# LSaldyt/JAX_llama

Measured on AMD Instinct MI355X. Metric: output_tokens_per_sec, higher is better.
Workload: dtype bf16; 1 GPU; model=llama3-8b, global_batch=2048, seq_len=384, prompt_len=128, gen_len=256, parallelism=dp1, mp=1

## Files before the change

### jax_llama_amd/csrc/bindings.cpp

```cpp
#include <torch/extension.h>
#include <c10/hip/HIPStream.h>

#include "kernels/launchers.h"

namespace {

using torch::Tensor;

hipStream_t stream() { return c10::hip::getCurrentHIPStream().stream(); }

void check(bool cond, const char* msg) { TORCH_CHECK(cond, "jax_llama_amd._C: ", msg); }

void check_gpu(const Tensor& t, const char* name) {
  TORCH_CHECK(t.is_cuda(), "jax_llama_amd._C: ", name, " must be a GPU tensor");
  TORCH_CHECK(t.is_contiguous(), "jax_llama_amd._C: ", name, " must be contiguous");
}

void rc(int r, const char* what) {
  TORCH_CHECK(r == 0, "jax_llama_amd._C: ", what, " failed (code ", r, ")");
}

void gemm_rc(int r, const char* what) {
  const char* why = r == -1   ? "no legal plan for this shape / tile id / epilogue / fused norm / K split"
                    : r == -3 ? "the slab workspace is missing or too small"
// ... 311 lines not shown
                     int64_t splits, c10::optional<Tensor> x_packed, int64_t spl, c10::optional<Tensor> sk_ws,
                     c10::optional<Tensor> sk_tk, c10::optional<Tensor> o_w, int64_t o_n, int64_t o_k,
                     c10::optional<Tensor> o_h, c10::optional<Tensor> o_hb, c10::optional<Tensor> o_hb_pack,
                     int64_t tp_state) {
  check_gpu(x, "x");
  check_packed(w, n, k);
  check(x.dim() == 2 && x.size(1) == k && x.scalar_type() == torch::kBFloat16, "linear_qkv_attn: x bf16 [M, K]");
  const int64_t m = x.size(0);
  check(m <= 32, "linear_qkv_attn: M <= 32");
  jla::QKVArgs qa = qkv_args(m, n, table, positions, kc, vc, slot, 1, h, hkv, dh, q);
  for (auto* t : {&kv_start, &out, &ws, &tickets, &sync}) check_gpu(*t, "linear_qkv_attn arg");
  check(kv_start.scalar_type() == torch::kInt32 && kv_start.numel() == m, "kv_start int32 [B]");
  check(out.scalar_type() == torch::kBFloat16 && out.numel() == m * h * dh, "out bf16 [B, H * Dh]");
  check(ws.scalar_type() == torch::kFloat32 && ws.numel() >= m * hkv * splits * (h / hkv) * (dh + 4), "ws too small");
  check(tickets.scalar_type() == torch::kInt32 && tickets.numel() >= m * hkv, "tickets int32 [pairs]");
  check(sync.scalar_type() == torch::kInt32 && (size_t)sync.numel() >= jla::qkv_attn_sync_ints(),
        "sync int32 [qkv_attn_sync_ints()]");
  check(t_cap <= kc.size(2), "t_cap <= cache length");
  const jla::bf16_t* xp = packed_ptr(x_packed, m, k, "x_packed");
  check(spl == 1 || spl == 2, "linear_qkv_attn: spl 1 or 2");
  if (spl > 1) {
    check(sk_ws.has_value() && sk_tk.has_value(), "linear_qkv_attn spl 2: sk_ws and sk_tk (skinny_workspace)");
    check_gpu(*sk_ws, "sk_ws");
    check_gpu(*sk_tk, "sk_tk");
    check(sk_ws->scalar_type() == torch::kFloat32 && sk_tk->scalar_type() == torch::kInt32 &&
              sk_tk->numel() >= n / 16,
          "linear_qkv_attn: sk_ws fp32, sk_tk int32 [N / 16]");
    qa.sk_ws = ptr<float>(*sk_ws);
    qa.sk_tk = ptr<int32_t>(*sk_tk);
    qa.sk_ws_floats = (int)sk_ws->numel();
  }
  jla::QKVArgs qo{};
  float* oh = nullptr;
  int o_mode = 0;
  if (o_w.has_value()) {
    check_packed(*o_w, o_n, o_k);
    check(o_k == h * dh, "linear_qkv_attn: Wo has H * Dh input columns");
    check(o_h.has_value() && o_hb.has_value(), "linear_qkv_attn: the fused o projection needs h and hb");
    check_gpu(*o_h, "h");
    check_gpu(*o_hb, "hb");
    check(o_h->scalar_type() == torch::kFloat32 && o_h->numel() == m * o_n && o_hb->scalar_type() == torch::kBFloat16 &&
              o_hb->numel() == m * o_n, "linear_qkv_attn: h fp32 / hb bf16 [M, N_o]");
    const int og = jla::qkv_attn_o_groups((int)m, (int)(h / hkv), (int)o_n, (int)o_k);
    check(og > 0, "linear_qkv_attn: the o projection cannot be fused at this shape (qkv_attn_o_groups)");
    oh = ptr<float>(*o_h);
    qo.res_bf16 = bf(*o_hb);
    qo.pack = packed_ptr(o_hb_pack, m, o_n, "o_hb_pack");
    o_mode = MODE_RESIDUAL;
    if (tp_state) {
      void* st = reinterpret_cast<void*>(tp_state);
      check(og <= jla::CAR_WG_COUNTERS && og * jla::TPRES_REGION <= jla::car_max_bytes(st),
            "linear_qkv_attn: too many o workgroups for the TP buffer");
      qo.tp = jla::car_device(st);
      o_mode = MODE_TPRESID;
    }
  }
  rc(jla::linear_qkv_attn(xp ? xp : cbf(x), w.data_ptr(), m, n, k, (float)rms_eps, qa, xp != nullptr, bf(out),
                          packed_ptr(out_pack, m, h * dh, "out_pack"), ptr<int32_t>(kv_start), ptr<float>(ws),
                          ptr<int32_t>(tickets), ptr<int32_t>(sync), (int)t_cap, (int)splits, (int)spl, stream(),
                          o_w.has_value() ? o_w->data_ptr() : nullptr, oh, (int)o_n, (int)o_k, o_mode,
                          o_w.has_value() ? &qo : nullptr),
     "linear_qkv_attn");
}

bool check_gemm_ws(const c10::optional<Tensor>& ws, int64_t k, int64_t ksplit, int64_t m, int64_t n, bool rms,
                   int64_t tile) {
  if (!is_g5(tile) && ksplit <= 1) return false;
  check(ws.has_value(), "gemm: a K split (gemm5: any plan) needs the slab workspace");
  check_gpu(*ws, "gemm ws");
  const int64_t ks = is_g5(tile) ? jla::gemm5_ksplit((int)k, (int)ksplit) : ksplit;
  check(ws->scalar_type() == torch::kFloat32 && ws->numel() >= ks * m * (n + (rms ? 1 : 0)), "gemm ws too small");
  return true;
}

static float* rms_ws_ptr(const c10::optional<Tensor>& rws, int64_t m, size_t* floats) {
  *floats = 0;
  if (!rws.has_value()) return nullptr;
  check_gpu(*rws, "rms_ws");
  check(rws->scalar_type() == torch::kFloat32 && rws->numel() >= m, "rms_ws: fp32, >= M floats");
  *floats = rws->numel();
  return ptr<float>(*rws);
}

void gemm(Tensor x, Tensor w, int64_t n, int64_t k, Tensor out, int64_t mode, bool accumulate,
          c10::optional<Tensor> mirror, int64_t ksplit, c10::optional<Tensor> ws, double rms_eps, int64_t tile,
          c10::optional<Tensor> pack_out, c10::optional<Tensor> rms_ws, int64_t n_body) {
  check_gpu(x, "x");
  check_packed(w, n, k);
  check(n_body >= 0 && (n_body == 0 || jla::gemm_tail_width((int)tile) > 0), "gemm n_body: tail-balanced tiles only");
  check(x.dim() == 2 && x.size(1) == k && x.scalar_type() == torch::kBFloat16, "x must be bf16 [M, K]");
  check(mode >= 0 && mode <= 2, "gemm mode");
  const int64_t m = x.size(0);
  check_linear_out(out, m, n, mode);
  jla::bf16_t* mir = mode == 1 ? mirror_ptr(mirror, out.numel()) : nullptr;
  jla::QKVArgs pqa{};
  if (pack_out.has_value()) {
    check(m <= SKINNY_MAX_M && (mode == 1 || mode == 2) && (mode != 1 || mir), "gemm pack_out: decode M, residual "
          "(with its mirror) or SwiGLU");
    check(ksplit > 1 || is_g5(tile), "gemm pack_out: the split-K reduce-kernel path only");
    pqa.pack = packed_ptr(pack_out, m, mode == 2 ? n / 2 : n, "pack_out");
  }
  const bool slabs = check_gemm_ws(ws, k, ksplit, m, n, rms_eps >= 0, tile);
  size_t rfl = 0;
  float* rws = rms_ws_ptr(rms_ws, m, &rfl);
  gemm_rc(jla::gemm(cbf(x), w.data_ptr(), out.data_ptr(), m, n, k, mode, accumulate,
                    out.scalar_type() == torch::kFloat32, mir, pqa.pack ? &pqa : nullptr,
                    slabs ? ptr<float>(*ws) : nullptr, slabs ? ws->numel() : 0, ksplit, stream(), (float)rms_eps,
                    (int)tile, rws, rfl, (int)n_body),
          "gemm");
}

void gemm_qkv(Tensor x, Tensor w, int64_t n, int64_t k, Tensor table, Tensor positions, Tensor kc, Tensor vc,
              Tensor slot, int64_t seq_len, int64_t h, int64_t hkv, int64_t dh, Tensor q, int64_t ksplit,
              c10::optional<Tensor> ws, double rms_eps, int64_t tile, c10::optional<Tensor> rms_ws) {
  check_gpu(x, "x");
  check_packed(w, n, k);
  check(x.dim() == 2 && x.size(1) == k && x.scalar_type() == torch::kBFloat16, "x must be bf16 [M, K]");
  const int64_t m = x.size(0);
  jla::QKVArgs qa = qkv_args(m, n, table, positions, kc, vc, slot, seq_len, h, hkv, dh, q);
  const bool slabs = check_gemm_ws(ws, k, ksplit, m, n, rms_eps >= 0, tile);
  size_t rfl = 0;
  float* rws = rms_ws_ptr(rms_ws, m, &rfl);
  gemm_rc(jla::gemm(cbf(x), w.data_ptr(), nullptr, m, n, k, MODE_QKV, 0, 0, nullptr, &qa,
                    slabs ? ptr<float>(*ws) : nullptr, slabs ? ws->numel() : 0, ksplit, stream(), (float)rms_eps,
                    (int)tile, rws, rfl),
          "gemm_qkv");
}

void rope_kv_write(Tensor qkv, Tensor table, Tensor positions, Tensor kc, Tensor vc, Tensor slot, int64_t seq_len,
                   int64_t h, int64_t hkv, int64_t dh, Tensor q) {
  for (auto* t : {&qkv, &table, &positions, &kc, &vc, &slot, &q}) check_gpu(*t, "rope_kv_write arg");
  check(qkv.scalar_type() == torch::kBFloat16 && kc.scalar_type() == torch::kBFloat16 &&
            vc.scalar_type() == torch::kBFloat16 && q.scalar_type() == torch::kBFloat16,
        "rope_kv_write bf16 tensors");
  check(table.scalar_type() == torch::kFloat32 && table.dim() == 3 && table.size(1) == dh / 2 && table.size(2) == 2,
        "rope table must be fp32 [L, Dh/2, 2]");
  check(positions.scalar_type() == torch::kInt32 && slot.scalar_type() == torch::kInt32, "int32 positions/slot");
  const int64_t m = qkv.size(0);
  check(qkv.dim() == 2 && qkv.size(1) == (h + 2 * hkv) * dh, "qkv shape");
  check(positions.numel() == m && m % seq_len == 0, "positions shape");
  const int64_t b = m / seq_len;
  check(kc.dim() == 4 && kc.size(0) == b && kc.size(1) == hkv && kc.size(3) == dh && vc.sizes() == kc.sizes(),
        "cache shape [B, Hkv, T, Dh]");
  check(q.numel() == m * h * dh, "q out shape");
  rc(jla::rope_kv_write(cbf(qkv), ptr<float>(table), table.size(0), ptr<int32_t>(positions), bf(kc), bf(vc),
                        ptr<int32_t>(slot), m, seq_len, h, hkv, dh, kc.size(2), bf(q), stream()),
     "rope_kv_write");
}

void check_attn(const Tensor& q, const Tensor& kc, const Tensor& vc, const Tensor& slot, const Tensor& kv_start,
                const c10::optional<Tensor>& key_mask, const Tensor& out) {
  for (auto* t : {&q, &kc, &vc, &slot, &kv_start, &out}) check_gpu(*t, "attention arg");
  check(q.scalar_type() == torch::kBFloat16 && kc.scalar_type() == torch::kBFloat16 &&
            vc.scalar_type() == torch::kBFloat16 && out.scalar_type() == torch::kBFloat16,
        "attention bf16 tensors");
  check(q.dim() == 4 && kc.dim() == 4 && kc.sizes() == vc.sizes(), "attention shapes");
  check(kc.size(0) == q.size(0) && kc.size(3) == q.size(3), "cache/q shape mismatch");
  check(q.size(2) % kc.size(1) == 0, "H must be a multiple of Hkv");
  check(slot.scalar_type() == torch::kInt32 && kv_start.scalar_type() == torch::kInt32 &&
            kv_start.numel() == q.size(0),
        "slot/kv_start");
  check(out.numel() == q.numel(), "attention out shape");
  if (key_mask.has_value()) {
    check_gpu(*key_mask, "key_mask");
    check(key_mask->scalar_type() == torch::kUInt8 && key_mask->dim() == 2 && key_mask->size(0) == q.size(0),
          "key_mask must be uint8 [B, L]");
  }
}

void attn_decode(Tensor q, Tensor kc, Tensor vc, Tensor slot, Tensor kv_start, c10::optional<Tensor> key_mask,
                 Tensor out, Tensor ws, Tensor tickets, int64_t t_cap, int64_t nsplit, c10::optional<Tensor> out_pack) {
  check_attn(q, kc, vc, slot, kv_start, key_mask, out);
  check(q.size(1) == 1, "attn_decode: one query per row");
  const int64_t b = q.size(0), h = q.size(2), dh = q.size(3), hkv = kc.size(1), T = kc.size(2);
  check(t_cap <= T, "t_cap exceeds the cache length");
  check_gpu(ws, "ws");
  check_gpu(tickets, "tickets");
  const jla::AttnPlanResult r = jla::attn_decode_plan(jla::attn_knobs(), b, h, hkv, dh, t_cap, key_mask.has_value());
  TORCH_CHECK(r.rc == 0, "jax_llama_amd._C: attn_decode: no plan (", r.why, "; see attn_plan.h)");
  TORCH_CHECK(nsplit == r.plan.nsplit, "jax_llama_amd._C: attn_decode: nsplit ", nsplit, " is not the plan's ",
              r.plan.nsplit, " (attn_decode_plan_check)");
  check(!out_pack.has_value() || r.plan.packs,
        "attn_decode: this launch does not write the packed copy (attn_decode_plan_check's packs)");
  check(ws.scalar_type() == torch::kFloat32 && (size_t)ws.numel() >= r.plan.ws_floats, "workspace too small");
  check(tickets.scalar_type() == torch::kInt32 && tickets.numel() >= r.plan.tickets, "tickets too small");
  const uint8_t* km = key_mask.has_value() ? ptr<uint8_t>(*key_mask) : nullptr;
  const int ml = key_mask.has_value() ? key_mask->size(1) : 0;
  rc(jla::attn_decode(cbf(q), cbf(kc), cbf(vc), ptr<int32_t>(slot), ptr<int32_t>(kv_start), km, ml, bf(out),
                      ptr<float>(ws), ptr<int32_t>(tickets), b, h, hkv, dh, T, t_cap, nsplit, stream(),
                      packed_ptr(out_pack, b, h * dh, "out_pack")),
     "attn_decode");
}

void attn_prefill(Tensor q, Tensor kc, Tensor vc, Tensor slot, Tensor kv_start, c10::optional<Tensor> key_mask,
                  Tensor out) {
  check_attn(q, kc, vc, slot, kv_start, key_mask, out);
  const uint8_t* km = key_mask.has_value() ? ptr<uint8_t>(*key_mask) : nullptr;
  const int ml = key_mask.has_value() ? key_mask->size(1) : 0;
  rc(jla::attn_prefill(cbf(q), cbf(kc), cbf(vc), ptr<int32_t>(slot), ptr<int32_t>(kv_start), km, ml, bf(out),
                       q.size(0), q.size(1), q.size(2), kc.size(1), q.size(3), kc.size(2), stream()),
     "attn_prefill");
}

void argmax(Tensor logits, Tensor idx, Tensor val) {
  check_gpu(logits, "logits");
  check_gpu(idx, "idx");
  check_gpu(val, "val");
  check(logits.scalar_type() == torch::kFloat32 && logits.dim() == 2, "logits must be fp32 [B, V]");
  check(idx.scalar_type() == torch::kInt32 && val.scalar_type() == torch::kFloat32 &&
            idx.numel() == logits.size(0) && val.numel() == logits.size(0),
        "argmax outputs");
  rc(jla::argmax(ptr<float>(logits), logits.size(0), logits.size(1), ptr<int32_t>(idx), ptr<float>(val), stream()),
     "argmax");
}

void gemm_argmax(Tensor x, Tensor w, int64_t n, int64_t k, Tensor ws, double rms_eps, Tensor idx, Tensor val,
                 c10::optional<Tensor> rms_ws) {
  check_gpu(x, "x");
  check_packed(w, n, k);
  check(x.dim() == 2 && x.size(1) == k && x.scalar_type() == torch::kBFloat16, "x must be bf16 [M, K]");
  const int64_t m = x.size(0);
  check_gpu(ws, "ws");
  check(ws.scalar_type() == torch::kFloat32 && (size_t)ws.numel() >= jla::gemm_argmax_workspace_floats(m, n),
        "gemm_argmax ws too small");
  check_gpu(idx, "idx");
  check_gpu(val, "val");
  check(idx.scalar_type() == torch::kInt32 && val.scalar_type() == torch::kFloat32 && idx.numel() == m &&
            val.numel() == m,
        "gemm_argmax outputs");
  size_t rfl = 0;
  float* rws = rms_ws_ptr(rms_ws, m, &rfl);
  rc(jla::gemm_argmax(cbf(x), w.data_ptr(), ptr<float>(ws), ws.numel(), m, n, k, (float)rms_eps, ptr<int32_t>(idx),
                      ptr<float>(val), stream(), rws, rfl),
     "gemm_argmax");
}

static void check_logprob_io(const Tensor& targets, const Tensor& tgt, const Tensor& mx, const Tensor& se, int64_t m,
                             int64_t col_offset) {
  for (auto* t : {&targets, &tgt, &mx, &se}) check_gpu(*t, "logprob arg");
  check(targets.scalar_type() == torch::kInt32 && targets.numel() == m, "targets must be int32 [M]");
  for (auto* t : {&tgt, &mx, &se})
    check(t->scalar_type() == torch::kFloat32 && t->numel() == m, "logprob outputs must be fp32 [M]");
  check(col_offset >= 0 && col_offset <= INT32_MAX, "col_offset");
}

void gemm_logprob(Tensor x, Tensor w, int64_t n, int64_t k, Tensor ws, double rms_eps, Tensor targets,
                  int64_t col_offset, Tensor tgt, Tensor mx, Tensor se, c10::optional<Tensor> rms_ws) {
  check_gpu(x, "x");
  check_packed(w, n, k);
  check(x.dim() == 2 && x.size(1) == k && x.scalar_type() == torch::kBFloat16, "x must be bf16 [M, K]");
  const int64_t m = x.size(0);
  check_gpu(ws, "ws");
  check(ws.scalar_type() == torch::kFloat32 && (size_t)ws.numel() >= jla::gemm_logprob_workspace_floats(m, n),
        "gemm_logprob ws too small");
  check_logprob_io(targets, tgt, mx, se, m, col_offset);
  size_t rfl = 0;
  float* rws = rms_ws_ptr(rms_ws, m, &rfl);
  gemm_rc(jla::gemm_logprob(cbf(x), w.data_ptr(), ptr<float>(ws), ws.numel(), m, n, k, (float)rms_eps,
                            ptr<int32_t>(targets), (int)col_offset, ptr<float>(tgt), ptr<float>(mx), ptr<float>(se),
                            stream(), rws, rfl),
          "gemm_logprob");
}

void logprob_rows(Tensor logits, Tensor targets, int64_t col_offset, Tensor tgt, Tensor mx, Tensor se) {
  check_gpu(logits, "logits");
  check(logits.scalar_type() == torch::kFloat32 && logits.dim() == 2 && logits.size(1) > 0,
        "logits must be fp32 [B, V]");
  check(logits.size(1) <= INT32_MAX, "logprob_rows: V too large");
  check_logprob_io(targets, tgt, mx, se, logits.size(0), col_offset);
  rc(jla::logprob_rows(ptr<float>(logits), logits.size(0), logits.size(1), ptr<int32_t>(targets), (int)col_offset,
                       ptr<float>(tgt), ptr<float>(mx), ptr<float>(se), stream()),
     "logprob_rows");
}

void topk_chunk(Tensor logits, int64_t k, int64_t idx_offset, Tensor cv, Tensor ci) {
  for (auto* t : {&logits, &cv, &ci}) check_gpu(*t, "topk_chunk arg");
  check(logits.scalar_type() == torch::kFloat32 && logits.dim() == 2, "logits must be fp32 [B, V]");
  const int64_t b = logits.size(0), v = logits.size(1);
  check(k >= 1 && k <= 64 && k <= v, "topk_chunk: 1 <= k <= min(64, V)");
  const int64_t c = (int64_t)jla::topk_chunks(v) * k;
  check(cv.scalar_type() == torch::kFloat32 && ci.scalar_type() == torch::kInt32 && cv.numel() == b * c &&
            ci.numel() == b * c,
        "topk_chunk: candidates must be [B, chunks*k] fp32/int32");
  rc(jla::topk_chunk(ptr<float>(logits), b, v, k, idx_offset, ptr<float>(cv), ptr<int32_t>(ci), stream()),
     "topk_chunk");
}

void topk_merge(Tensor cv, Tensor ci, int64_t k, int64_t mode, c10::optional<Tensor> out_v,
                c10::optional<Tensor> out_i, c10::optional<Tensor> nxt, double temperature, double top_p,
                int64_t seed, c10::optional<Tensor> step) {
  check_gpu(cv, "cv");
  check_gpu(ci, "ci");
  check(cv.dim() == 2 && cv.sizes() == ci.sizes() && cv.scalar_type() == torch::kFloat32 &&
            ci.scalar_type() == torch::kInt32,
        "topk_merge: candidates [B, C] fp32/int32");
  const int64_t b = cv.size(0), c = cv.size(1);
  check(k >= 1 && k <= 64 && k <= c && c <= 4096, "topk_merge: 1 <= k <= 64, k <= C <= 4096");
  float* ov = nullptr;
  int32_t* oi = nullptr;
  int32_t* nx = nullptr;
  const int32_t* st = nullptr;
  if (mode == 0) {
    check(out_v.has_value() && out_i.has_value(), "topk_merge mode 0 needs out_v/out_i");
    check_gpu(*out_v, "out_v");
    check_gpu(*out_i, "out_i");
    check(out_v->scalar_type() == torch::kFloat32 && out_i->scalar_type() == torch::kInt32 &&
              out_v->numel() == b * k && out_i->numel() == b * k,
          "topk_merge outputs [B, k]");
    ov = ptr<float>(*out_v);
    oi = ptr<int32_t>(*out_i);
  } else {
    check(mode == 1 && nxt.has_value() && step.has_value(), "topk_merge mode 1 needs nxt and step");
    check_gpu(*nxt, "nxt");
    check_gpu(*step, "step");
    check(nxt->scalar_type() == torch::kInt32 && nxt->numel() == b && step->scalar_type() == torch::kInt32,
          "topk_merge nxt [B] / step [1] int32");
// ... 90 lines not shown
  check(m >= 1 && m <= SKINNY_MAX_M, "linear_tp_residual: 1 <= M <= 64");
  check(h.scalar_type() == torch::kFloat32 && h.numel() == m * n && hb.scalar_type() == torch::kBFloat16 &&
            hb.numel() == m * n, "h fp32 / hb bf16 [M, N]");
  void* st = reinterpret_cast<void*>(state);
  const int64_t groups = n / 16;
  check(groups <= jla::CAR_WG_COUNTERS && groups * jla::TPRES_REGION <= jla::car_max_bytes(st),
        "linear_tp_residual: too many workgroups for the buffer");
  jla::QKVArgs qa{};
  qa.res_bf16 = bf(hb);
  qa.pack = packed_ptr(hb_pack, m, n, "hb_pack");
  qa.tp = jla::car_device(st);
  run_skinny(x, w, n, k, h.data_ptr(), MODE_TPRESID, -1.0, true, true, &qa, variant, ws ? *ws : Tensor(),
             tickets ? *tickets : Tensor(), packed_ptr(x_packed, m, k, "x_packed"));
}

void gemm_tp_residual(int64_t state, Tensor x, Tensor w, int64_t n, int64_t k, Tensor h, Tensor hb, int64_t ksplit,
                      Tensor ws, int64_t tile) {
  check_gpu(x, "x");
  check_gpu(h, "h");
  check_gpu(hb, "hb");
  check_packed(w, n, k);
  check(x.dim() == 2 && x.size(1) == k && x.scalar_type() == torch::kBFloat16, "x must be bf16 [M, K]");
  const int64_t m = x.size(0);
  check(h.scalar_type() == torch::kFloat32 && h.numel() == m * n && hb.scalar_type() == torch::kBFloat16 &&
            hb.numel() == m * n, "h fp32 / hb bf16 [M, N]");
  void* st = reinterpret_cast<void*>(state);
  const int64_t groups = jla::gemm_tp_groups((int)m, (int)n);
  check(groups <= jla::CAR_WG_COUNTERS && groups * jla::TPRES_REGION <= jla::car_max_bytes(st),
        "gemm_tp_residual: the output does not fit the fused exchange buffer");
  check_gemm_ws(ws, k, ksplit, m, n, false, tile);
  jla::QKVArgs qa{};
  qa.tp = jla::car_device(st);
  gemm_rc(jla::gemm(cbf(x), w.data_ptr(), h.data_ptr(), m, n, k, MODE_TPRESID, 1, 1, bf(hb), &qa, ptr<float>(ws),
                    ws.numel(), ksplit, stream(), -1.f, (int)tile, nullptr, 0),
          "gemm_tp_residual");
}

void car_pairs(int64_t state, int64_t mode, Tensor vals, Tensor idx, int64_t idx_offset, int64_t k,
               c10::optional<Tensor> out_v, Tensor out_i) {
  check_gpu(vals, "vals");
  check_gpu(idx, "idx");
  check_gpu(out_i, "out_i");
  check(vals.scalar_type() == torch::kFloat32 && idx.scalar_type() == torch::kInt32 &&
            out_i.scalar_type() == torch::kInt32 && vals.numel() == idx.numel(),
        "car_pairs dtypes");
  const int64_t n = vals.numel();
  auto* st = reinterpret_cast<void*>(state);
  float* ov = nullptr;
  if (out_v.has_value()) {
    check_gpu(*out_v, "out_v");
    check(out_v->scalar_type() == torch::kFloat32 && out_v->numel() == out_i.numel(), "out_v");
    ov = ptr<float>(*out_v);
  }
  if (mode == 0) {
    check(out_i.numel() == n, "car_pairs argmax out shape");
  } else {
    check(mode == 1 && ov && k > 0 && n % k == 0 && out_i.numel() == n * jla::car_world(st), "car_pairs top-k shapes");
  }
  rc(jla::car_pairs(st, (int)mode, ptr<float>(vals), ptr<int32_t>(idx), (int)idx_offset, n, (int)k, ov,
                    ptr<int32_t>(out_i), stream()),
     "car_pairs");
}

}

PYBIND11_MODULE(TORCH_EXTENSION_NAME, m) {
  m.doc() = "jax_llama_amd gfx950 (MI355X) HIP kernels";
  m.attr("SKINNY_MAX_M") = SKINNY_MAX_M;
  m.attr("ARCH") = "gfx950";
  m.def("embedding", &embedding, py::arg("ids"), py::arg("table"), py::arg("out"),
        py::arg("mirror") = py::none());
  m.def("rms_scale", &rms_scale);
  m.def("rmsnorm", &rmsnorm);
  m.def("residual_add", &residual_add);
  m.def("gemm_f32", &gemm_f32);
  m.def("prefetch", &prefetch, py::arg("t"), py::arg("grid") = 128);
  m.def("linear_skinny", &linear_skinny, py::arg("x"), py::arg("w"), py::arg("n"), py::arg("k"), py::arg("out"),
        py::arg("mode"), py::arg("rms_eps"), py::arg("accumulate"), py::arg("variant"), py::arg("ws"),
        py::arg("tickets"), py::arg("mirror") = py::none(), py::arg("x_packed") = py::none(),
        py::arg("pack_out") = py::none());
  m.def("gemm", &gemm, py::arg("x"), py::arg("w"), py::arg("n"), py::arg("k"), py::arg("out"), py::arg("mode"),
        py::arg("accumulate"), py::arg("mirror") = py::none(), py::arg("ksplit") = 1, py::arg("ws") = py::none(),
        py::arg("rms_eps") = -1.0, py::arg("tile") = 0, py::arg("pack_out") = py::none(),
        py::arg("rms_ws") = py::none(), py::arg("n_body") = 0);
  m.def("gemm_tail_split", [](int64_t tiles_m, int64_t n, int64_t width, int64_t cus) {
    const int nb = jla::gemm_tail_split((int)tiles_m, (int)n, (int)width, cus > 0 ? (int)cus : jla::gemm_num_cus());
    return std::make_pair((int64_t)nb, nb > 0 ? (n - nb * width + 127) / 128 : (int64_t)0);
  }, py::arg("tiles_m"), py::arg("n"), py::arg("width"), py::arg("cus") = 0);
  m.def("gemm_plan_check", [](int64_t m, int64_t n, int64_t k, int64_t mode, bool rms, int64_t ksplit, int64_t tile,
                              bool has_rms_ws, int64_t n_body) {
    return jla::gemm_plan_check((int)m, (int)n, (int)k, (int)mode, rms, (int)ksplit, (int)tile, has_rms_ws, (int)n_body);
  }, py::arg("m"), py::arg("n"), py::arg("k"), py::arg("mode"), py::arg("rms"), py::arg("ksplit"), py::arg("tile"),
     py::arg("has_rms_ws"), py::arg("n_body") = 0);
  m.def("gemv_plan_check", [](int64_t m, int64_t n, int64_t k, int64_t mode, bool x_f32, bool x_packed,
                              int64_t variant) {
    const jla::GemvPlanResult r = jla::gemv_plan((int)m, (int)n, (int)k, (int)mode, x_f32, x_packed, (int)variant);
    const jla::GemvPlan& p = r.plan;
    return py::make_tuple(r.rc, p.mt, p.nt, p.nw, p.deep, p.xp, p.ksplit);
  }, py::arg("m"), py::arg("n"), py::arg("k"), py::arg("mode"), py::arg("x_f32"), py::arg("x_packed"),
     py::arg("variant"));
  m.def("gemv_w8_plan_check", [](int64_t m, int64_t n, int64_t k, int64_t mode, bool x_f32) {
    const jla::GemvPlanResult r = jla::gemv_w8_plan((int)m, (int)n, (int)k, (int)mode, x_f32);
    return py::make_tuple(r.rc, r.plan.mt, r.plan.nt, r.plan.nw);
  }, py::arg("m"), py::arg("n"), py::arg("k"), py::arg("mode"), py::arg("x_f32"));
  m.def("dequant_fp8", &dequant_fp8, py::arg("w8"), py::arg("scale"), py::arg("n"), py::arg("k"), py::arg("out"));
  m.def("linear_skinny_w8", &linear_skinny_w8, py::arg("x"), py::arg("w8"), py::arg("scale"), py::arg("n"),
        py::arg("k"), py::arg("out"), py::arg("mode"), py::arg("rms_eps"), py::arg("accumulate"),
        py::arg("mirror") = py::none(), py::arg("pack_out") = py::none());
  m.def("linear_qkv_w8", &linear_qkv_w8, py::arg("x"), py::arg("w8"), py::arg("scale"), py::arg("n"), py::arg("k"),
        py::arg("rms_eps"), py::arg("table"), py::arg("positions"), py::arg("kc"), py::arg("vc"), py::arg("slot"),
        py::arg("seq_len"), py::arg("h"), py::arg("hkv"), py::arg("dh"), py::arg("q"));
  m.def("gemv_variant_table", []() {
    py::dict t;
    for (const jla::GemvVariant& v : jla::GEMV_VARIANTS) t[py::int_(v.id)] = py::make_tuple(v.xp, v.split);
    return t;
  });
  m.attr("GEMV_SPLIT_MAX_GROUPS") = jla::GEMV_SPLIT_MAX_GROUPS;
  m.def("gemm_qkv_direct_ok", [](int64_t m, int64_t tile, int64_t k) {
    return jla::gemm_qkv_direct_ok((int)m, (int)tile, (int)k) != 0;
  });
  m.def("gemm_set_g4_default", [](int64_t on) { jla::gemm_set_g4_default((int)on); });
  m.def("gemm_set_g4_group", [](int64_t gm) { jla::gemm_set_g4_group((int)gm); });
  m.def("gemm_qkv", &gemm_qkv, py::arg("x"), py::arg("w"), py::arg("n"), py::arg("k"), py::arg("table"),
        py::arg("positions"), py::arg("kc"), py::arg("vc"), py::arg("slot"), py::arg("seq_len"), py::arg("h"),
        py::arg("hkv"), py::arg("dh"), py::arg("q"), py::arg("ksplit"), py::arg("ws"), py::arg("rms_eps") = -1.0,
        py::arg("tile") = 0, py::arg("rms_ws") = py::none());
  m.def("gemm_argmax", &gemm_argmax, py::arg("x"), py::arg("w"), py::arg("n"), py::arg("k"), py::arg("ws"),
        py::arg("rms_eps"), py::arg("idx"), py::arg("val"), py::arg("rms_ws") = py::none());
  m.def("gemm_argmax_workspace", [](int64_t m, int64_t n) { return (int64_t)jla::gemm_argmax_workspace_floats(m, n); });
  m.def("gemm_logprob", &gemm_logprob, py::arg("x"), py::arg("w"), py::arg("n"), py::arg("k"), py::arg("ws"),
        py::arg("rms_eps"), py::arg("targets"), py::arg("col_offset"), py::arg("tgt"), py::arg("mx"), py::arg("se"),
        py::arg("rms_ws") = py::none());
  m.def("gemm_logprob_workspace",
        [](int64_t m, int64_t n) { return (int64_t)jla::gemm_logprob_workspace_floats(m, n); });
  m.def("logprob_rows", &logprob_rows);
  m.def("gemm_ksplit", [](int64_t m, int64_t n, int64_t k) { return jla::gemm_ksplit(m, n, k); });
  m.def("rope_kv_write", &rope_kv_write);
  m.def("attn_set_impl", [](int64_t impl, int64_t waves_target) { jla::attn_set_impl(impl, waves_target); },
        py::arg("impl"), py::arg("waves_target") = 0);
  m.def("attn_reset_knobs", []() { jla::attn_reset_knobs(); }, "every attn_set_* knob back to its default");
  m.def("attn_decode_plan_check", [](int64_t b, int64_t h, int64_t hkv, int64_t dh, int64_t t_cap, bool masked) {
    const jla::AttnPlanResult r =
        jla::attn_decode_plan(jla::attn_knobs(), (int)b, (int)h, (int)hkv, (int)dh, (int)t_cap, masked);
    const jla::AttnPlan& p = r.plan;
    return py::make_tuple(r.rc, r.why, r.rc ? "" : jla::attn_kernel_name(p.kernel), p.nsplit, p.packs,
                          (int64_t)p.ws_floats, p.tickets, p.rep, p.kpg, p.ring, p.fold, p.wpp, p.split_len);
  }, py::arg("b"), py::arg("h"), py::arg("hkv"), py::arg("dh"), py::arg("t_cap"), py::arg("masked"));
  m.def("attn_decode_splits", [](int64_t b, int64_t hkv, int64_t t, int64_t rep) {
    return jla::attn_decode_plan(jla::attn_knobs(), (int)b, (int)(hkv * rep), (int)hkv, jla::ATTN_DH, (int)t, false)
        .plan.nsplit;
  });
  m.def("attn_decode_packs", [](int64_t b, int64_t hkv, int64_t rep) {
    return (int)jla::attn_decode_plan(jla::attn_knobs(), (int)b, (int)(hkv * rep), (int)hkv, jla::ATTN_DH, 1, false)
        .plan.packs;
  });
  m.def("linear_qkv", &linear_qkv, py::arg("x"), py::arg("w"), py::arg("n"), py::arg("k"), py::arg("rms_eps"),
        py::arg("table"), py::arg("positions"), py::arg("kc"), py::arg("vc"), py::arg("slot"), py::arg("seq_len"),
        py::arg("h"), py::arg("hkv"), py::arg("dh"), py::arg("q"), py::arg("variant"), py::arg("ws"), py::arg("tickets"),
        py::arg("x_packed") = py::none());
  m.def("linear_qkv_attn", &linear_qkv_attn, py::arg("x"), py::arg("w"), py::arg("n"), py::arg("k"),
        py::arg("rms_eps"), py::arg("table"), py::arg("positions"), py::arg("kc"), py::arg("vc"), py::arg("slot"),
        py::arg("h"), py::arg("hkv"), py::arg("dh"), py::arg("q"), py::arg("kv_start"), py::arg("out"),
        py::arg("out_pack"), py::arg("ws"), py::arg("tickets"), py::arg("sync"), py::arg("t_cap"), py::arg("splits"),
        py::arg("x_packed") = py::none(), py::arg("spl") = 1, py::arg("sk_ws") = py::none(),
        py::arg("sk_tk") = py::none(), py::arg("o_w") = py::none(), py::arg("o_n") = 0, py::arg("o_k") = 0,
        py::arg("o_h") = py::none(), py::arg("o_hb") = py::none(), py::arg("o_hb_pack") = py::none(),
        py::arg("tp_state") = 0);
  m.def("qkv_attn_splits", [](int64_t m, int64_t b, int64_t hkv, int64_t rep, int64_t t_cap, int64_t n, int64_t cus,
                              int64_t spl, int64_t o_groups) {
    return jla::qkv_attn_splits((int)m, (int)b, (int)hkv, (int)rep, (int)t_cap, (int)n, (int)cus, (int)spl,
                                (int)o_groups);
  }, py::arg("m"), py::arg("b"), py::arg("hkv"), py::arg("rep"), py::arg("t_cap"), py::arg("n"), py::arg("cus"),
     py::arg("spl") = 1, py::arg("o_groups") = 0);
  m.def("qkv_attn_o_groups", [](int64_t m, int64_t rep, int64_t n, int64_t k) {
    return jla::qkv_attn_o_groups((int)m, (int)rep, (int)n, (int)k);
  });
  m.def("qkv_attn_sync_ints", []() { return (int64_t)jla::qkv_attn_sync_ints(); });
  m.def("qkv_attn_set_o_nt", [](int64_t nt) { jla::qkv_attn_set_o_nt((int)nt); });
  m.def("qkv_attn_set_diag", [](int64_t d) { jla::qkv_attn_set_diag((int)d); });
  m.def("qkv_attn_set_stamps", [](c10::optional<Tensor> t) {
    if (t.has_value()) {
      check_gpu(*t, "stamps");
      check(t->scalar_type() == torch::kInt64, "stamps int64");
    }
    jla::qkv_attn_set_stamps(t.has_value() ? reinterpret_cast<unsigned long long*>(t->data_ptr()) : nullptr);
  });
  m.def("qkv_attn_occupancy", [](int64_t m, int64_t rep, int64_t spl, int64_t o_groups) {
    return jla::qkv_attn_occupancy((int)m, (int)rep, (int)spl, (int)o_groups);
  }, py::arg("m"), py::arg("rep"), py::arg("spl") = 1, py::arg("o_groups") = 0);
  m.def("skinny_workspace", &skinny_workspace);
  m.def("linear_skinny_argmax", &linear_skinny_argmax);
  m.def("gemm_tp_residual", &gemm_tp_residual, py::arg("state"), py::arg("x"), py::arg("w"), py::arg("n"), py::arg("k"),
        py::arg("h"), py::arg("hb"), py::arg("ksplit"), py::arg("ws"), py::arg("tile"));
  m.def("gemm_tp_groups", [](int64_t m, int64_t n) { return (int64_t)jla::gemm_tp_groups((int)m, (int)n); });
  m.def("linear_tp_residual", &linear_tp_residual, py::arg("state"), py::arg("x"), py::arg("w"), py::arg("n"),
        py::arg("k"), py::arg("h"), py::arg("hb"), py::arg("variant"), py::arg("x_packed") = py::none(),
        py::arg("hb_pack") = py::none(), py::arg("ws") = py::none(), py::arg("tickets") = py::none());
  m.def("bounds_error", [](bool reset) {
    const int r = reset ? 1 : 0;
    return (int64_t)(jla::jla_bounds_norm_embed(r) | jla::jla_bounds_rope_kv(r) | jla::jla_bounds_sample(r) |
                     jla::jla_bounds_gemm(r) | jla::jla_bounds_gemv(r) |
                     jla::jla_bounds_attn_decode(r) | jla::jla_bounds_attn_prefill(r));
  }, "OR of the bounds-checked debug build's error words (JLA_BOUNDS_* bits); always 0 in a release build",
        py::arg("reset") = false);
#ifdef JLA_DEBUG_BOUNDS
  m.attr("DEBUG_BOUNDS") = true;
#else
  m.attr("DEBUG_BOUNDS") = false;
#endif
  m.def("attn_set_diag", [](int64_t d) { jla::attn_set_diag((int)d); });
  m.def("cu_mask_stream", [](std::vector<int64_t> words) {
// ... 66 lines not shown
```

### jax_llama_amd/csrc/kernels/common.h

```cpp
#pragma once
#include <hip/hip_runtime.h>
#include <stdint.h>

#include "gemm_plan.h"

typedef uint16_t bf16_t;
typedef __bf16 bf16x8_t __attribute__((ext_vector_type(8)));
typedef short s16x8 __attribute__((ext_vector_type(8)));
typedef float f32x4 __attribute__((ext_vector_type(4)));
typedef unsigned int u32x4 __attribute__((ext_vector_type(4)));
typedef unsigned int u32x2 __attribute__((ext_vector_type(2)));

#define JLA_BOUNDS_TOKEN 0
#define JLA_BOUNDS_KV_SLOT 1
#define JLA_BOUNDS_SEQ 2
#define JLA_BOUNDS_ATTN_T 3
#define JLA_BOUNDS_ROPE_POS 4
#ifdef JLA_DEBUG_BOUNDS
static __device__ unsigned int g_jla_bounds_err;
#define JLA_FLAG(code) atomicOr(&g_jla_bounds_err, 1u << (code))
#define JLA_BOUNDS_ACCESSOR(tu)                                                     \
  unsigned jla_bounds_##tu(int reset) {                                             \
    unsigned v = 0;                                                                 \
    (void)hipMemcpyFromSymbol(&v, HIP_SYMBOL(g_jla_bounds_err), sizeof(v));         \
// ... 8 lines not shown
#define JLA_BOUNDS_ACCESSOR(tu) \
  unsigned jla_bounds_##tu(int) { return 0; }
#endif

#define JLA_DEV __device__ __forceinline__

JLA_DEV float bf2f(bf16_t v) { return __uint_as_float(((uint32_t)v) << 16); }

typedef __bf16 bf16x2_t __attribute__((ext_vector_type(2)));
typedef float f32x2_t __attribute__((ext_vector_type(2)));

JLA_DEV bf16_t f2bf(float f) { return __builtin_bit_cast(bf16_t, (__bf16)f); }

JLA_DEV uint32_t pack2bf(float lo, float hi) {
  const f32x2_t v = {lo, hi};
  return __builtin_bit_cast(uint32_t, __builtin_convertvector(v, bf16x2_t));
}

JLA_DEV void unpack8(const u32x4 v, float* f) {
#pragma unroll
  for (int i = 0; i < 4; ++i) {
    f[2 * i] = __uint_as_float(v[i] << 16);
    f[2 * i + 1] = __uint_as_float(v[i] & 0xffff0000u);
  }
}

JLA_DEV u32x4 pack8(const float* f) {
  u32x4 r;
#pragma unroll
  for (int i = 0; i < 4; ++i) r[i] = pack2bf(f[2 * i], f[2 * i + 1]);
  return r;
}

JLA_DEV float dot8_bf16(const u32x4 a, const u32x4 b, float acc) {
  const bf16x8_t x = __builtin_bit_cast(bf16x8_t, a), y = __builtin_bit_cast(bf16x8_t, b);
  acc = __builtin_amdgcn_fdot2_f32_bf16(__builtin_shufflevector(x, x, 0, 1), __builtin_shufflevector(y, y, 0, 1), acc, false);
  acc = __builtin_amdgcn_fdot2_f32_bf16(__builtin_shufflevector(x, x, 2, 3), __builtin_shufflevector(y, y, 2, 3), acc, false);
  acc = __builtin_amdgcn_fdot2_f32_bf16(__builtin_shufflevector(x, x, 4, 5), __builtin_shufflevector(y, y, 4, 5), acc, false);
  acc = __builtin_amdgcn_fdot2_f32_bf16(__builtin_shufflevector(x, x, 6, 7), __builtin_shufflevector(y, y, 6, 7), acc, false);
  return acc;
}

JLA_DEV size_t pack_off(int m, int k, int K) {
  return ((size_t)((m >> 4) * (K >> 5) + (k >> 5)) * 64 + (m & 15) + 16 * ((k & 31) >> 3)) * 8 + (k & 7);
}

JLA_DEV f32x4 mfma16x16x32(const u32x4 a, const u32x4 b, f32x4 c) {
  return __builtin_amdgcn_mfma_f32_16x16x32_bf16(__builtin_bit_cast(bf16x8_t, a),
                                                 __builtin_bit_cast(bf16x8_t, b), c, 0, 0, 0);
}

JLA_DEV void glds16(const void* gsrc, void* lds_wave_base) {
  __builtin_amdgcn_global_load_lds((const __attribute__((address_space(1))) void*)gsrc,
                                   (__attribute__((address_space(3))) void*)lds_wave_base, 16, 0, 0);
}
#pragma clang diagnostic push
#pragma clang diagnostic ignored "-Winline-asm"
JLA_DEV void glds16_asm(const void* gsrc, void* lds_wave_base) {
  const unsigned m0 = __builtin_amdgcn_readfirstlane(
      (unsigned)(size_t)(__attribute__((address_space(3))) char*)lds_wave_base);
  asm volatile("s_mov_b32 m0, %1\n\ts_nop 0\n\tglobal_load_lds_dwordx4 %0, off" ::"v"(gsrc), "s"(m0) : "memory", "m0");
}
#pragma clang diagnostic pop
template <int N>
JLA_DEV void wait_vmcnt() {
  static_assert(N >= 0 && N < 64, "vmcnt range");
  __builtin_amdgcn_s_waitcnt(0xF70 | (N & 15) | ((N >> 4) << 14));
}

JLA_DEV u32x4 load_nt(const u32x4* p) { return __builtin_nontemporal_load(p); }

JLA_DEV float wave_sum(float v) {
#pragma unroll
  for (int o = 32; o > 0; o >>= 1) v += __shfl_xor(v, o, 64);
  return v;
}

JLA_DEV float wave_max(float v) {
#pragma unroll
  for (int o = 32; o > 0; o >>= 1) v = fmaxf(v, __shfl_xor(v, o, 64));
  return v;
}

JLA_DEV float block_sum(float v, float* red) {
  const int lane = threadIdx.x & 63, wid = threadIdx.x >> 6, nw = (blockDim.x + 63) >> 6;
  v = wave_sum(v);
  __syncthreads();
  if (lane == 0) red[wid] = v;
  __syncthreads();
  float s = 0.f;
  for (int i = 0; i < nw; ++i) s += red[i];
  return s;
}

JLA_DEV float silu(float x) { return x / (1.f + __expf(-x)); }

template <int CTRL>
JLA_DEV float dppf(float v) {
  return __builtin_bit_cast(float, __builtin_amdgcn_update_dpp(0, __builtin_bit_cast(int, v), CTRL, 0xF, 0xF, false));
}
JLA_DEV float row16_sum(float v) {
  v += dppf<0xB1>(v);
  v += dppf<0x4E>(v);
  v += dppf<0x141>(v);
  v += dppf<0x140>(v);
  return v;
}

#define JLA_CHECK_LAUNCH()                                                        \
  do {                                                                            \
    hipError_t e__ = hipGetLastError();                                           \
    if (e__ != hipSuccess) return (int)e__;                                       \
  } while (0)
```

### jax_llama_amd/csrc/kernels/gemm.hip

```cpp
#include <type_traits>

#include "car.h"
#include "common.h"
#include "gemm4w.h"
#include "gemm5ws.h"
#include "gemm_plan.h"
#include "launchers.h"
#include "ring.h"

namespace jla {

constexpr int G2_BN = 256, G2_NBUF = 4, G2_GROUP_M = 8;
#ifdef JLA_GEMM_STAMPS
__device__ unsigned long long g_gemm_stamps[8192 * 8 * 6];
#endif

JLA_DEV void g2_tile_coords(int pid, int tiles_m, int tiles_n, int& tm, int& tn) {
  const int in_group = G2_GROUP_M * tiles_n;
  const int first_m = (pid / in_group) * G2_GROUP_M;
  const int gsz = min(tiles_m - first_m, G2_GROUP_M);
  tm = first_m + (pid % in_group) % gsz;
  tn = (pid % in_group) / gsz;
}

// ... 966 lines not shown
  }
  const size_t idx = e4 * 4;
  const int m = (int)(idx / N), col = (int)(idx - (size_t)m * N);
  float4 v = sum_splits(ws, ksplit, slab4, e4);
  float rs = 1.f;
  if (ssq) {
    float t = 0.f;
    for (int s = 0; s < ksplit; ++s) t += ssq[(size_t)s * M + m];
    rs = 1.f / sqrtf(t / (float)K + rms_eps);
    v.x *= rs;
    v.y *= rs;
    v.z *= rs;
    v.w *= rs;
  }
  float vv[4] = {v.x, v.y, v.z, v.w};
  if constexpr (MODE == MODE_SWIGLU) {
    const int tile = col >> 4, c0 = col & 15;
    float4 u = sum_splits(ws, ksplit, slab4, e4 + 4);
    u.x *= rs;
    u.y *= rs;
    u.z *= rs;
    u.w *= rs;
    const float uu[4] = {u.x, u.y, u.z, u.w};
    bf16_t* o = static_cast<bf16_t*>(out) + (size_t)m * (N >> 1) + (tile >> 1) * 16 + c0;
    const uint2 pk = make_uint2(pack2bf(silu(vv[0]) * uu[0], silu(vv[1]) * uu[1]),
                                pack2bf(silu(vv[2]) * uu[2], silu(vv[3]) * uu[3]));
    *reinterpret_cast<uint2*>(o) = pk;
    if (qa.pack) *reinterpret_cast<uint2*>(qa.pack + pack_off(m, (tile >> 1) * 16 + c0, N >> 1)) = pk;
  } else if constexpr (MODE == MODE_RESIDUAL) {
    float4* o = reinterpret_cast<float4*>(static_cast<float*>(out) + idx);
    float4 r = *o;
    if (accumulate) {
      r.x += vv[0];
      r.y += vv[1];
      r.z += vv[2];
      r.w += vv[3];
    } else {
      r = make_float4(vv[0], vv[1], vv[2], vv[3]);
    }
    *o = r;
    if (mirror) {
      const uint2 pk = make_uint2(pack2bf(r.x, r.y), pack2bf(r.z, r.w));
      *reinterpret_cast<uint2*>(mirror + idx) = pk;
      if (qa.pack) *reinterpret_cast<uint2*>(qa.pack + pack_off(m, col, N)) = pk;
    }
  } else if constexpr (MODE == MODE_QKV) {
    const int head = col / qa.Dh, d0 = col - head * qa.Dh;
    const int b = m / qa.S, sq = m - b * qa.S;
    if (head < qa.H + qa.Hkv) {
      int pos = qa.positions[m];
      if (pos < 0 || pos >= qa.table_len) JLA_FLAG(JLA_BOUNDS_ROPE_POS);
      pos = pos < 0 ? 0 : (pos >= qa.table_len ? qa.table_len - 1 : pos);
#pragma unroll
      for (int p = 0; p < 2; ++p) {
        const float2 cs = qa.table[(size_t)pos * (qa.Dh >> 1) + (d0 >> 1) + p];
        const float xr = vv[2 * p], xi = vv[2 * p + 1];
        vv[2 * p] = xr * cs.x - xi * cs.y;
        vv[2 * p + 1] = xr * cs.y + xi * cs.x;
      }
    }
    const uint2 packed = make_uint2(pack2bf(vv[0], vv[1]), pack2bf(vv[2], vv[3]));
    if (head < qa.H) {
      *reinterpret_cast<uint2*>(qa.q + ((size_t)m * qa.H + head) * qa.Dh + d0) = packed;
    } else {
      const int slot = qa.slot[0] + sq;
      if (slot < qa.T) {
        const bool is_k = head < qa.H + qa.Hkv;
        const int kh = is_k ? head - qa.H : head - qa.H - qa.Hkv;
        bf16_t* cache = is_k ? qa.kc : qa.vc;
        *reinterpret_cast<uint2*>(cache + (((size_t)b * qa.Hkv + kh) * qa.T + slot) * qa.Dh + d0) = packed;
      } else {
        JLA_FLAG(JLA_BOUNDS_KV_SLOT);
      }
    }
  } else {
    if (out_f32)
      *reinterpret_cast<float4*>(static_cast<float*>(out) + idx) = make_float4(vv[0], vv[1], vv[2], vv[3]);
    else
      *reinterpret_cast<uint2*>(static_cast<bf16_t*>(out) + idx) =
          make_uint2(pack2bf(vv[0], vv[1]), pack2bf(vv[2], vv[3]));
  }
}

constexpr int TPR_ELEMS = 4096;
static_assert(TPR_ELEMS / 2 * 8 == TPRES_REGION, "one fused-exchange region per workgroup");
__global__ void __launch_bounds__(256)
    gemm_reduce_tp_kernel(const float* __restrict__ ws, int ksplit, float* __restrict__ h, bf16_t* __restrict__ hb,
                          int M, int N, const CarDevice* __restrict__ dev) {
  const CarDevice& d = *dev;
  const int w = blockIdx.x;
  const size_t slab4 = (size_t)M * N / 4;
  __shared__ int s_calls;
  if (threadIdx.x == 0) s_calls = __hip_atomic_load(d.wg_ctr + w, __ATOMIC_RELAXED, __HIP_MEMORY_SCOPE_AGENT) + 1;
  u32x2 gq[4];
  f32x4 hv[4];
#pragma unroll
  for (int j = 0; j < 4; ++j) {
    const size_t e4 = (size_t)w * (TPR_ELEMS / 4) + j * 256 + threadIdx.x;
    gq[j] = u32x2{0u, 0u};
    hv[j] = f32x4{0.f, 0.f, 0.f, 0.f};
    if (e4 < slab4) {
      const float4 v = sum_splits(ws, ksplit, slab4, e4);
      gq[j] = u32x2{pack2bf(v.x, v.y), pack2bf(v.z, v.w)};
      hv[j] = *reinterpret_cast<const f32x4*>(h + e4 * 4);
    }
  }
  __syncthreads();
  const int calls = s_calls;
  const unsigned tag = gran_tag_fused(calls);
  const long long wg_base = (long long)w * TPRES_REGION;
  const long long par_base = (long long)(calls & 1) * d.world * d.max_bytes;
#pragma unroll
  for (int j = 0; j < 4; ++j) {
    const size_t e4 = (size_t)w * (TPR_ELEMS / 4) + j * 256 + threadIdx.x;
    if (e4 >= slab4) continue;
    const long long g = wg_base + (long long)(j * 256 + threadIdx.x) * 16;
    for (int p = 0; p < d.world; ++p) {
      const __amdgpu_buffer_rsrc_t rp = rsrc(d.buf[p]);
      const long long o = par_base + (long long)d.rank * d.max_bytes + g;
      st_sys8(rp, o, u32x2{gq[j][0], tag});
      st_sys8(rp, o + 8, u32x2{gq[j][1], tag});
    }
  }
  const bool give_up = __hip_atomic_load(d.error, __ATOMIC_RELAXED, __HIP_MEMORY_SCOPE_SYSTEM) != 0;
  const __amdgpu_buffer_rsrc_t mine = rsrc(d.buf[d.rank]);
#pragma unroll
  for (int j = 0; j < 4; ++j) {
    const size_t e4 = (size_t)w * (TPR_ELEMS / 4) + j * 256 + threadIdx.x;
    if (e4 >= slab4) continue;
    const long long g = wg_base + (long long)(j * 256 + threadIdx.x) * 16;
    float sm[4] = {0.f, 0.f, 0.f, 0.f};
    u32x4 r[CAR_MAX_WORLD];
    car_gather16(d, mine, par_base + g, d.max_bytes, tag, give_up, r);
#pragma unroll
    for (int p = 0; p < CAR_MAX_WORLD; ++p) {
      if (p < d.world) {
        sm[0] += __uint_as_float(r[p][0] << 16);
        sm[1] += __uint_as_float(r[p][0] & 0xffff0000u);
        sm[2] += __uint_as_float(r[p][2] << 16);
        sm[3] += __uint_as_float(r[p][2] & 0xffff0000u);
      }
    }
    f32x4 n;
#pragma unroll
    for (int i = 0; i < 4; ++i) n[i] = hv[j][i] + sm[i];
    *reinterpret_cast<f32x4*>(h + e4 * 4) = n;
    *reinterpret_cast<u32x2*>(hb + e4 * 4) = u32x2{pack2bf(n[0], n[1]), pack2bf(n[2], n[3])};
  }
  if (threadIdx.x == 0) __hip_atomic_store(d.wg_ctr + w, calls, __ATOMIC_RELAXED, __HIP_MEMORY_SCOPE_AGENT);
}
int gemm_tp_groups(int M, int N) { return (int)(((size_t)M * N + TPR_ELEMS - 1) / TPR_ELEMS); }


static int g2_wm(int M) { return M <= 128 ? 1 : 2; }

int gemm_ksplit(int M, int N, int K) {
  const int KS = K >> 5;
  const int bm = 128 * g2_wm(M);
  const int tiles = ((N + G2_BN - 1) / G2_BN) * ((M + bm - 1) / bm);
  int ks = min(256 / tiles, max(1, K / (2 * M)));
  ks = ks < 1 ? 1 : (ks > 16 ? 16 : ks);
  while (ks > 1 && KS / ks < 4) --ks;
  const int kc = (KS + ks - 1) / ks;
  return (KS + kc - 1) / kc;
}

size_t gemm_workspace_floats(int M, int N, int K) {
  const int ks = gemm_ksplit(M, N, K);
  return ks > 1 ? (size_t)ks * M * (N + 1) : 0;
}

static int num_cus() {
  static int cus = 0;
  if (cus == 0) {
    int dev = 0;
    hipDeviceProp_t prop;
    if (hipGetDevice(&dev) == hipSuccess && hipGetDeviceProperties(&prop, dev) == hipSuccess)
      cus = prop.multiProcessorCount;
    if (cus <= 0) cus = 256;
  }
  return cus;
}
int gemm_num_cus() { return num_cus(); }

static bool g_g4_default = true;
void gemm_set_g4_default(int on) { g_g4_default = on != 0; }
int gemm_qkv_direct_ok(int M, int tile, int K) {
  const GemmPlanResult r = gemm_plan(M, 16, K, MODE_QKV, true, 1, tile, true, 0, 0, g_g4_default);
  return r.rc == 0 && !r.plan.reduce;
}
int gemm_plan_check(int M, int N, int K, int mode, int rms, int ksplit, int tile, int has_rms_ws, int n_body) {
  return gemm_plan(M, N, K, mode, rms != 0, ksplit, tile, has_rms_ws != 0, n_body, num_cus(), g_g4_default).rc;
}

struct GemmArgs {
  const bf16_t* x;
  const u32x4* w;
  void* out;
  int M, N, K, accumulate, out_f32;
  bf16_t* mirror;
  float rms_eps;
  float* ssq;
  float* rms_ws;
  QKVArgs qa;
  hipStream_t s;
};

static bool g4_row_stat(const GemmArgs& a, const GemmPlan& p, const float*& inv) {
  inv = p.norm == NORM_PRECOMPUTED ? a.rms_ws : nullptr;
  return inv == nullptr || rms_rowinv(a.x, a.rms_ws, a.M, a.K, a.rms_eps, a.s) == 0;
}

static int g_g4_group = 0;
void gemm_set_g4_group(int gm) { g_g4_group = gm; }
static int g4_group_m(int tiles_m) {
  const int gm = g_g4_group > 0 ? g_g4_group : 4;
  return gm < tiles_m ? gm : tiles_m;
}
static int g_g5_diag = 0;
void gemm5_set_diag(int d) { g_g5_diag = d; }

template <int MODE, int NJ>
static void launch_g4(const GemmArgs& a, const GemmPlan& p) {
  const int tm = (a.M + G4_BM - 1) / G4_BM, tn = (a.N + 32 * NJ - 1) / (32 * NJ);
  const int grid = tm * tn * p.ksplit, gm = g4_group_m(tm);
  const float* inv;
  if (!g4_row_stat(a, p, inv)) return;
#define JLA_G4(R, DIAG, DEEP)                                                                                       \
  gemm4_kernel<MODE, R, NJ, DIAG, DEEP><<<grid, 256, 0, a.s>>>(a.x, a.w, a.out, a.M, a.N, a.K, a.accumulate, a.out_f32, \
                                                               a.mirror, p.kc, tm, tn, a.rms_eps, a.ssq, a.qa, inv, gm)
  if constexpr (NJ != 8) {
    if (inv)
      JLA_G4(2, 0, true);
    else
      JLA_G4(0, 0, true);
  } else {
    if constexpr (MODE == MODE_STORE) {
      if (p.norm == NORM_NONE && (g_g5_diag & 192)) {
        if ((g_g5_diag & 192) == 64)
          JLA_G4(0, 1, false);
        else if ((g_g5_diag & 192) == 128)
          JLA_G4(0, 2, false);
        else
          JLA_G4(0, 3, false);
        return;
      }
    }
    if (p.norm == NORM_PRECOMPUTED) {
      if (p.deep) JLA_G4(2, 0, true); else JLA_G4(2, 0, false);
    } else if (p.norm == NORM_INLOOP) {
      if (p.deep) JLA_G4(1, 0, true); else JLA_G4(1, 0, false);
    } else {
      if (p.deep) JLA_G4(0, 0, true); else JLA_G4(0, 0, false);
    }
  }
#undef JLA_G4
}

template <int MODE>
static void launch_g4p(const GemmArgs& a, const GemmPlan& p) {
  const int tm = (a.M + G4_BM - 1) / G4_BM, tn = (a.N + G4_BN - 1) / G4_BN;
  const int grid = min(tm * tn, num_cus()), gm = g4_group_m(tm);
  const float* inv;
  if (!g4_row_stat(a, p, inv)) return;
#define JLA_G4P(R)                                                                                                  \
  gemm4p_kernel<MODE, R><<<grid, 256, 0, a.s>>>(a.x, a.w, a.out, a.M, a.N, a.K, a.accumulate, a.out_f32, a.mirror, tm, \
                                                tn, a.rms_eps, a.qa, inv, gm)
  if (p.norm == NORM_PRECOMPUTED)
    JLA_G4P(2);
  else if (p.norm == NORM_INLOOP)
    JLA_G4P(1);
  else
    JLA_G4P(0);
#undef JLA_G4P
}

template <int MODE, int NJB>
static void launch_g4t(const GemmArgs& a, const GemmPlan& p) {
  const int tm = (a.M + G4_BM - 1) / G4_BM, nt = (a.N - p.n_body * 32 * NJB + 127) / 128;
  const int grid = tm * (p.n_body + nt), gm = g4_group_m(tm);
  const float* inv;
  if (!g4_row_stat(a, p, inv)) return;
  if (inv)
    gemm4t_kernel<MODE, 2, NJB><<<grid, 256, 0, a.s>>>(a.x, a.w, a.out, a.M, a.N, a.K, a.accumulate, a.out_f32,
                                                       a.mirror, tm, p.n_body, nt, a.rms_eps, inv, gm);
  else
    gemm4t_kernel<MODE, 0, NJB><<<grid, 256, 0, a.s>>>(a.x, a.w, a.out, a.M, a.N, a.K, a.accumulate, a.out_f32,
                                                       a.mirror, tm, p.n_body, nt, a.rms_eps, nullptr, gm);
}

template <int MODE>
static void launch_g2(const GemmArgs& a, const GemmPlan& p) {
  const int cfg = p.family;
// ... 7 lines not shown
  if (cfg == 2)                              \
    JLA_G2(1, false, R, 8, 4, false, 0);     \
  else if (cfg == 3)                         \
    JLA_G2(2, true, R, 4, 2, false, 0);      \
  else                                       \
    JLA_G2(2, true, R, 8, 4, true, 2)
  [[maybe_unused]] const bool rms = p.norm != NORM_NONE;
  if constexpr (MODE == MODE_QKV) {
    JLA_G2(2, true, true, 8, 4, true, 2);
  } else if constexpr (MODE == MODE_ARGMAX) {
    if (rms)
      JLA_G2(2, true, true, 8, 4, true, 2);
    else
      JLA_G2(2, true, false, 8, 4, true, 2);
  } else if constexpr (MODE == MODE_RESIDUAL) {
    JLA_G2_CFG(false);
  } else {
    if (rms) {
      JLA_G2_CFG(true);
    } else {
      JLA_G2_CFG(false);
    }
  }
#undef JLA_G2_CFG
#undef JLA_G2
}

static void launch_g5(const GemmArgs& a, const GemmPlan& p) {
  const int mt = a.M <= 128 ? 8 : 16, rows = 16 * mt, ntw = p.nj;
  const int tiles_m = (a.M + rows - 1) / rows, tiles_n = (a.N + 64 * ntw - 1) / (64 * ntw);
  const int grid = tiles_m * tiles_n * p.ksplit;
#define JLA_G5(MTV, NTV)                                                                                            \
  gemm5_partial_kernel<MTV, NTV><<<grid, 256, 0, a.s>>>(a.x, a.w, static_cast<float*>(a.out), a.M, a.N, a.K, p.kc, \
                                                        tiles_m, tiles_n, a.ssq, g_g5_diag)
  if (mt == 8 && ntw == 4)
    JLA_G5(8, 4);
  else if (mt == 8)
    JLA_G5(8, 2);
  else if (ntw == 4)
    JLA_G5(16, 4);
  else
    JLA_G5(16, 2);
#undef JLA_G5
}

template <int MODE>
static void launch_plan(const GemmArgs& a, const GemmPlan& p) {
  constexpr bool PLAIN = MODE == MODE_STORE || MODE == MODE_RESIDUAL || MODE == MODE_SWIGLU;
  switch (p.family) {
    case GEMM2_256x256:
    case GEMM2_128x256:
    case GEMM2_128x128:
      if constexpr (MODE != MODE_LOGPROB) launch_g2<MODE>(a, p);
      break;
    case GEMM4:
      if (p.nj == 8) launch_g4<MODE, 8>(a, p);
      if constexpr (MODE != MODE_ARGMAX && MODE != MODE_LOGPROB) {
        if (p.nj == 6) launch_g4<MODE, 6>(a, p);
      }
      if constexpr (PLAIN || MODE == MODE_PARTIAL) {
        if (p.nj == 4) launch_g4<MODE, 4>(a, p);
      }
      break;
    case GEMM4_PERSISTENT:
      if constexpr (PLAIN || MODE == MODE_QKV) launch_g4p<MODE>(a, p);
      break;
    case GEMM4_TAIL:
      if constexpr (PLAIN) {
        if (p.nj == 6)
          launch_g4t<MODE, 6>(a, p);
        else
          launch_g4t<MODE, 8>(a, p);
      }
      break;
    case GEMM5:
      if constexpr (MODE == MODE_PARTIAL) launch_g5(a, p);
      break;
    case GEMM_NONE: break;
  }
}

static int launch_reduce(const float* ws, int ksplit, void* out, int M, int N, int K, int mode, int accumulate,
                         int out_f32, bf16_t* mirror, const QKVArgs* qkv, const float* ssq, float rms_eps,
                         hipStream_t s) {
  const size_t total4 = (size_t)M * N / (mode == MODE_SWIGLU ? 8 : 4);
  const int rgrid = (int)((total4 + 255) / 256);
  QKVArgs qa{};
  if (qkv) qa = *qkv;
  const float eps = ssq ? rms_eps : 0.f;
  switch (mode) {
    case MODE_STORE:
      gemm_reduce_kernel<MODE_STORE><<<rgrid, 256, 0, s>>>(ws, ksplit, out, M, N, accumulate, out_f32, nullptr, qa,
                                                           ssq, K, eps);
      break;
    case MODE_RESIDUAL:
      gemm_reduce_kernel<MODE_RESIDUAL><<<rgrid, 256, 0, s>>>(ws, ksplit, out, M, N, accumulate, 1, mirror, qa,
                                                              nullptr, K, eps);
      break;
    case MODE_SWIGLU:
      gemm_reduce_kernel<MODE_SWIGLU><<<rgrid, 256, 0, s>>>(ws, ksplit, out, M, N, accumulate, 0, nullptr, qa, ssq,
                                                            K, eps);
      break;
    case MODE_QKV:
      gemm_reduce_kernel<MODE_QKV><<<rgrid, 256, 0, s>>>(ws, ksplit, out, M, N, accumulate, 0, nullptr, qa, ssq, K,
                                                         eps);
      break;
    case MODE_TPRESID:
      if (!qkv || !qa.tp || !mirror || ssq || (N & 3)) return -1;
      gemm_reduce_tp_kernel<<<gemm_tp_groups(M, N), 256, 0, s>>>(ws, ksplit, static_cast<float*>(out), mirror, M, N,
                                                                 static_cast<const CarDevice*>(qa.tp));
      break;
    default: return -1;
  }
  JLA_CHECK_LAUNCH();
  return 0;
}

int gemm(const bf16_t* x, const void* W, void* out, int M, int N, int K, int mode, int accumulate, int out_f32,
         bf16_t* mirror, const QKVArgs* qkv, float* ws, size_t ws_floats, int ksplit, hipStream_t s,
         float rms_eps, int tile, float* rms_ws, size_t rms_ws_floats, int n_body) {
  const bool has_rms_ws = rms_ws != nullptr && rms_ws_floats >= (size_t)M;
  const GemmPlanResult r =
      gemm_plan(M, N, K, mode, rms_eps >= 0.f, ksplit, tile, has_rms_ws, n_body, num_cus(), g_g4_default);
  const GemmPlan& p = r.plan;
  if (r.rc != 0 || p.family == GEMM_NONE) return r.rc;
  if (mode == MODE_ARGMAX || mode == MODE_LOGPROB || (mode == MODE_QKV && !qkv)) return -1;
  const u32x4* w = static_cast<const u32x4*>(W);
  if (!p.reduce) {
    GemmArgs a{x, w, out, M, N, K, accumulate, out_f32, nullptr, rms_eps, nullptr, rms_ws, QKVArgs{}, s};
    switch (mode) {
      case MODE_QKV:
        a.out = nullptr, a.accumulate = a.out_f32 = 0, a.qa = *qkv;
        launch_plan<MODE_QKV>(a, p);
        break;
      case MODE_STORE: launch_plan<MODE_STORE>(a, p); break;
      case MODE_RESIDUAL:
        a.out_f32 = 1, a.mirror = mirror, a.rms_eps = -1.f;
        launch_plan<MODE_RESIDUAL>(a, p);
        break;
      case MODE_SWIGLU:
        a.out_f32 = 0;
        launch_plan<MODE_SWIGLU>(a, p);
        break;
      default: return -1;
    }
    JLA_CHECK_LAUNCH();
    return 0;
  }
  const size_t slabs = (size_t)p.ksplit * M * N;
  if (ws == nullptr || ws_floats < slabs + (p.norm != NORM_NONE ? (size_t)p.ksplit * M : 0)) return -3;
  float* ssq = p.norm != NORM_NONE ? ws + slabs : nullptr;
  launch_plan<MODE_PARTIAL>(GemmArgs{x, w, ws, M, N, K, 0, 1, nullptr, rms_eps, ssq, nullptr, QKVArgs{}, s}, p);
  JLA_CHECK_LAUNCH();
  return launch_reduce(ws, p.ksplit, out, M, N, K, mode, accumulate, out_f32, mirror, qkv, ssq, rms_eps, s);
}

JLA_DEV void amax_merge(float& bv, int& bi, float ov, int oi) {
  if (ov > bv || (ov == bv && oi < bi)) {
    bv = ov;
    bi = oi;
  }
}

template <int TPR>
__global__ void __launch_bounds__(TPR == 64 ? 256 : TPR)
    argmax_partials_kernel(const float2* __restrict__ part, int P, int M, int32_t* __restrict__ idx,
                           float* __restrict__ val) {
  __shared__ float s_v[16];
  __shared__ int s_i[16];
  const int row = TPR == 64 ? blockIdx.x * 4 + (threadIdx.x >> 6) : blockIdx.x;
  const int t = TPR == 64 ? (threadIdx.x & 63) : threadIdx.x;
  if (row >= M) return;
  const float2* pr = part + (size_t)row * P;
  float bv[4] = {-INFINITY, -INFINITY, -INFINITY, -INFINITY};
  int bi[4] = {0x7fffffff, 0x7fffffff, 0x7fffffff, 0x7fffffff};
  for (int k0 = t; k0 < P; k0 += 4 * TPR) {
    float2 e[4];
#pragma unroll
    for (int u = 0; u < 4; ++u) {
      const int k = k0 + u * TPR;
      e[u] = k < P ? pr[k] : make_float2(-INFINITY, __int_as_float(0x7fffffff));
    }
#pragma unroll
    for (int u = 0; u < 4; ++u) amax_merge(bv[u], bi[u], e[u].x, __float_as_int(e[u].y));
  }
#pragma unroll
  for (int u = 1; u < 4; ++u) amax_merge(bv[0], bi[0], bv[u], bi[u]);
#pragma unroll
  for (int o = 32; o > 0; o >>= 1) amax_merge(bv[0], bi[0], __shfl_xor(bv[0], o, 64), __shfl_xor(bi[0], o, 64));
  if constexpr (TPR > 64) {
    const int w = threadIdx.x >> 6;
    if ((threadIdx.x & 63) == 0) {
      s_v[w] = bv[0];
      s_i[w] = bi[0];
    }
    __syncthreads();
    if (threadIdx.x == 0) {
      for (int ww = 1; ww < TPR / 64; ++ww) amax_merge(bv[0], bi[0], s_v[ww], s_i[ww]);
      idx[row] = bi[0] == 0x7fffffff ? 0 : bi[0];
      val[row] = bv[0];
    }
  } else if (t == 0) {
    idx[row] = bi[0] == 0x7fffffff ? 0 : bi[0];
    val[row] = bv[0];
  }
}

static void launch_argmax_partials(const float2* part, int P, int M, int32_t* idx, float* val, hipStream_t s) {
  if (M <= 512)
    argmax_partials_kernel<1024><<<M, 1024, 0, s>>>(part, P, M, idx, val);
  else
    argmax_partials_kernel<64><<<(M + 3) / 4, 256, 0, s>>>(part, P, M, idx, val);
}

int argmax_partials(const float* part, int P, int M, int32_t* idx, float* val, hipStream_t s) {
  if (M <= 0) return 0;
  launch_argmax_partials(reinterpret_cast<const float2*>(part), P, M, idx, val, s);
  JLA_CHECK_LAUNCH();
  return 0;
}

size_t gemm_argmax_workspace_floats(int M, int N) { return (size_t)M * ((N + G2_BN - 1) / G2_BN) * 4 * 2; }

int gemm_argmax(const bf16_t* x, const void* W, float* ws, size_t ws_floats, int M, int N, int K, float rms_eps,
                int32_t* idx, float* val, hipStream_t s, float* rms_ws, size_t rms_ws_floats) {
  const bool has_rms_ws = rms_ws != nullptr && rms_ws_floats >= (size_t)M;
  const GemmPlanResult r = gemm_plan(M, N, K, MODE_ARGMAX, rms_eps >= 0.f, 1, 0, has_rms_ws, 0, 0, g_g4_default);
  if (r.rc != 0 || r.plan.family == GEMM_NONE) return r.rc;
  if (ws == nullptr || ws_floats < gemm_argmax_workspace_floats(M, N)) return -3;
  launch_plan<MODE_ARGMAX>(
      GemmArgs{x, static_cast<const u32x4*>(W), ws, M, N, K, 0, 1, nullptr, rms_eps, nullptr, rms_ws, QKVArgs{}, s},
      r.plan);
  JLA_CHECK_LAUNCH();
  const int P = (N + G2_BN - 1) / G2_BN * (r.plan.family == GEMM4 ? 2 : 4);
  launch_argmax_partials(reinterpret_cast<const float2*>(ws), P, M, idx, val, s);
  JLA_CHECK_LAUNCH();
  return 0;
}

JLA_DEV void lse_merge(float& m, float& s, float om, float os) {
  constexpr float LOG2E = 1.4426950408889634f;
  if (om == -INFINITY) return;
  if (m == -INFINITY) {
    m = om;
    s = os;
    return;
  }
  const float nm = fmaxf(m, om);
  s = s * __builtin_amdgcn_exp2f((m - nm) * LOG2E) + os * __builtin_amdgcn_exp2f((om - nm) * LOG2E);
  m = nm;
}

template <int TPR>
__global__ void __launch_bounds__(TPR == 64 ? 256 : TPR)
    lse_partials_kernel(const float2* __restrict__ part, int P, int M, float* __restrict__ mx,
                        float* __restrict__ se) {
  __shared__ float s_m[16];
  __shared__ float s_s[16];
  const int row = TPR == 64 ? blockIdx.x * 4 + (threadIdx.x >> 6) : blockIdx.x;
  const int t = TPR == 64 ? (threadIdx.x & 63) : threadIdx.x;
  if (row >= M) return;
  const float2* pr = part + (size_t)row * P;
  float bm[4] = {-INFINITY, -INFINITY, -INFINITY, -INFINITY};
  float bs[4] = {0.f, 0.f, 0.f, 0.f};
  for (int k0 = t; k0 < P; k0 += 4 * TPR) {
    float2 e[4];
#pragma unroll
    for (int u = 0; u < 4; ++u) {
      const int k = k0 + u * TPR;
      e[u] = k < P ? pr[k] : make_float2(-INFINITY, 0.f);
    }
#pragma unroll
    for (int u = 0; u < 4; ++u) lse_merge(bm[u], bs[u], e[u].x, e[u].y);
  }
#pragma unroll
  for (int u = 1; u < 4; ++u) lse_merge(bm[0], bs[0], bm[u], bs[u]);
#pragma unroll
  for (int o = 32; o > 0; o >>= 1)
    lse_merge(bm[0], bs[0], __shfl_xor(bm[0], o, 64), __shfl_xor(bs[0], o, 64));
  if constexpr (TPR > 64) {
    const int w = threadIdx.x >> 6;
    if ((threadIdx.x & 63) == 0) {
      s_m[w] = bm[0];
      s_s[w] = bs[0];
    }
    __syncthreads();
    if (threadIdx.x == 0) {
      for (int ww = 1; ww < TPR / 64; ++ww) lse_merge(bm[0], bs[0], s_m[ww], s_s[ww]);
      mx[row] = bm[0];
      se[row] = bs[0];
    }
  } else if (t == 0) {
    mx[row] = bm[0];
    se[row] = bs[0];
  }
}

static void launch_lse_partials(const float2* part, int P, int M, float* mx, float* se, hipStream_t s) {
  if (M <= 512)
    lse_partials_kernel<1024><<<M, 1024, 0, s>>>(part, P, M, mx, se);
  else
    lse_partials_kernel<64><<<(M + 3) / 4, 256, 0, s>>>(part, P, M, mx, se);
}

size_t gemm_logprob_workspace_floats(int M, int N) { return (size_t)M * ((N + G4_BN - 1) / G4_BN) * 2 * 2; }

int gemm_logprob(const bf16_t* x, const void* W, float* ws, size_t ws_floats, int M, int N, int K, float rms_eps,
                 const int32_t* targets, int col_offset, float* tgt, float* mx, float* se, hipStream_t s,
                 float* rms_ws, size_t rms_ws_floats) {
  const bool has_rms_ws = rms_ws != nullptr && rms_ws_floats >= (size_t)M;
  const GemmPlanResult r = gemm_plan(M, N, K, MODE_LOGPROB, rms_eps >= 0.f, 1, 0, has_rms_ws, 0, 0, g_g4_default);
  if (r.rc != 0 || r.plan.family == GEMM_NONE) return r.rc;
  if (ws == nullptr || ws_floats < gemm_logprob_workspace_floats(M, N)) return -3;
  if (targets == nullptr || tgt == nullptr || mx == nullptr || se == nullptr) return -1;
  const hipError_t zeroed = hipMemsetAsync(tgt, 0, (size_t)M * sizeof(float), s);
// ... 14 lines not shown
```

### jax_llama_amd/csrc/kernels/launchers.h

```cpp
#pragma once
#include <hip/hip_runtime.h>
#include <stdint.h>

#include "attn_plan.h"
#include "gemm_plan.h"
#include "gemv_plan.h"

namespace jla {
typedef uint16_t bf16_t;

int embedding(const int32_t* ids, const bf16_t* table, float* out, bf16_t* mirror, int M, int D, int V,
              hipStream_t s);
int rms_scale(const float* x, bf16_t* out, int M, int D, float eps, hipStream_t s);
int rms_scale_bf16(const bf16_t* x, bf16_t* out, int M, int D, float eps, hipStream_t s);
int rms_rowinv(const bf16_t* x, float* inv, int M, int D, float eps, hipStream_t s);
int residual_add(float* h, const void* p, int p_bf16, bf16_t* hb, long long n, hipStream_t s);
int prefetch(const void* p, long long nbytes, int grid, unsigned* sink, hipStream_t s);
int stream_probe(const void* p, long long nbytes, int grid, unsigned* sink, hipStream_t s);
int gemm_f32(const float* x, const float* w, float* y, int M, int N, int K, hipStream_t s);
int rmsnorm(const float* x, const float* w, float* out, int M, int D, float eps, hipStream_t s);

struct QKVArgs {
  const float2* table;
  int table_len;
  union {
    const int32_t* positions;
    const int32_t* lp_targets;
  };
  bf16_t* kc;
  bf16_t* vc;
  const int32_t* slot;
  int S, H, Hkv, Dh, T;
  bf16_t* q;
  bf16_t* res_bf16;
  bf16_t* pack;
  const void* tp;
  union {
    float* sk_ws;
    float* lp_tgt;
  };
  int32_t* sk_tk;
  union {
    int sk_ws_floats;
    int lp_col_offset;
  };
};

constexpr int CAR_WG_COUNTERS = 4096;
constexpr long long TPRES_REGION = 64 * 64 * 4;

int qkv_attn_o_groups(int M, int rep, int N, int K);
size_t qkv_attn_sync_ints();
void qkv_attn_set_o_nt(int nt);
int qkv_attn_splits(int M, int B, int Hkv, int rep, int t_cap, int N, int cus, int spl = 1, int o_groups = 0);
int qkv_attn_occupancy(int M, int rep, int spl = 1, int o_groups = 0);
void qkv_attn_set_stamps(unsigned long long* p);
void qkv_attn_set_diag(int d);
int linear_qkv_attn(const bf16_t* x, const void* W, int M, int N, int K, float rms_eps, const QKVArgs& qa, bool xp,
                    bf16_t* out, bf16_t* out_pack, const int32_t* kv_start, float* ws, int32_t* tickets, int32_t* sync,
                    int t_cap, int splits, int spl, hipStream_t s,
                    const void* o_w = nullptr, float* o_h = nullptr, int o_n = 0, int o_k = 0, int o_mode = 0,
                    const QKVArgs* qo = nullptr);
int linear_skinny(const void* x, int x_is_f32, const void* W, void* out, int M, int N, int K, int mode,
                  float rms_eps, int accumulate, int out_f32, const QKVArgs* qkv, int variant, hipStream_t s);
int dequant_fp8(const void* W8, const float* scale, void* out, int N, int K, hipStream_t s);
int linear_skinny_w8(const void* x, int x_is_f32, const void* W8, const float* scale, void* out, int M, int N, int K,
                     int mode, float rms_eps, int accumulate, int out_f32, const QKVArgs* qkv, hipStream_t s);
int clock_probe(int iters, int grid, unsigned long long* out, hipStream_t s);
int gemm(const bf16_t* x, const void* W, void* out, int M, int N, int K, int mode, int accumulate, int out_f32,
         bf16_t* mirror, const QKVArgs* qkv, float* ws, size_t ws_floats, int ksplit, hipStream_t s,
         float rms_eps = -1.f, int tile = 0, float* rms_ws = nullptr, size_t rms_ws_floats = 0, int n_body = 0);
int gemm_plan_check(int M, int N, int K, int mode, int rms, int ksplit, int tile, int has_rms_ws, int n_body);
int gemm_ksplit(int M, int N, int K);
size_t gemm_workspace_floats(int M, int N, int K);
int gemm_tp_groups(int M, int N);
int gemm_qkv_direct_ok(int M, int tile, int K);
int gemm_num_cus();
void gemm_set_g4_default(int on);
void gemm_set_g4_group(int gm);
void gemm5_set_diag(int d);
int gemm_argmax(const bf16_t* x, const void* W, float* ws, size_t ws_floats, int M, int N, int K, float rms_eps,
                int32_t* idx, float* val, hipStream_t s, float* rms_ws = nullptr, size_t rms_ws_floats = 0);
size_t gemm_argmax_workspace_floats(int M, int N);
int argmax_partials(const float* part, int P, int M, int32_t* idx, float* val, hipStream_t s);
int gemm_logprob(const bf16_t* x, const void* W, float* ws, size_t ws_floats, int M, int N, int K, float rms_eps,
                 const int32_t* targets, int col_offset, float* tgt, float* mx, float* se, hipStream_t s,
                 float* rms_ws = nullptr, size_t rms_ws_floats = 0);
size_t gemm_logprob_workspace_floats(int M, int N);

int rope_kv_write(const bf16_t* qkv, const float* table, int table_len, const int32_t* positions, bf16_t* kc,
                  bf16_t* vc, const int32_t* slot, int M, int S, int H, int Hkv, int Dh, int T, bf16_t* q_out,
                  hipStream_t s);

const AttnKnobs& attn_knobs();
void attn_reset_knobs();
void attn_set_impl(int impl, int waves_target);
void attn_set_v3_max_pairs(int n);
void attn_set_v3_kpg(int mult);
void attn_set_v5_max_pairs(int n);
void attn_set_v5_fold(int n);
void attn_set_v6(int mode);
void attn_set_v6_wpp(int wpp);
void attn_set_diag(int d);
void attn_set_v6_diag(int d);
unsigned jla_bounds_norm_embed(int reset);
unsigned jla_bounds_rope_kv(int reset);
unsigned jla_bounds_sample(int reset);
unsigned jla_bounds_gemm(int reset);
unsigned jla_bounds_gemv(int reset);
unsigned jla_bounds_attn_decode(int reset);
unsigned jla_bounds_attn_prefill(int reset);
int attn_decode(const bf16_t* q, const bf16_t* kc, const bf16_t* vc, const int32_t* slot, const int32_t* kv_start,
                const uint8_t* key_mask, int mask_len, bf16_t* out, float* ws, int32_t* tickets, int B, int H,
                int Hkv, int Dh, int T, int t_cap, int nsplit, hipStream_t s, bf16_t* out_pack = nullptr);
int attn_decode_v6(const bf16_t* q, const bf16_t* kc, const bf16_t* vc, const int32_t* slot, const int32_t* kv_start,
                   const uint8_t* key_mask, int mask_len, bf16_t* out, int B, int H, int Hkv, int T, int t_cap,
                   int wpp, hipStream_t s, bf16_t* out_pack);
void attn_prefill_set_impl(int impl);
int attn_prefill(const bf16_t* q, const bf16_t* kc, const bf16_t* vc, const int32_t* slot, const int32_t* kv_start,
                 const uint8_t* key_mask, int mask_len, bf16_t* out, int B, int S, int H, int Hkv, int Dh, int T,
                 hipStream_t s);

int argmax(const float* logits, int B, int V, int32_t* idx, float* val, hipStream_t s);
int logprob_rows(const float* logits, int B, int V, const int32_t* targets, int col_offset, float* tgt, float* mx,
                 float* se, hipStream_t s);
int topk_chunks(int V);
int topk_chunk(const float* logits, int B, int V, int K, int idx_offset, float* cv, int32_t* ci, hipStream_t s);
int topk_merge(const float* cv, const int32_t* ci, int B, int C, int K, int mode, float* out_v, int32_t* out_i,
               int32_t* nxt, float temperature, float top_p, uint64_t seed, const int32_t* step, hipStream_t s);
size_t car_buffer_bytes(long long max_bytes, int world);
int car_alloc(long long max_bytes, int world, void** buf, void** sig, hipIpcMemHandle_t* hbuf, hipIpcMemHandle_t* hsig);
void car_free(void* buf, void* sig);
int car_init(int rank, int world, long long max_bytes, void* own_buf, void* own_sig, const hipIpcMemHandle_t* hbufs,
             const hipIpcMemHandle_t* hsigs, double timeout_s, void** state);
int car_reduce(void* state, int op, const void* in, void* out, float* h, bf16_t* hb, long long nbytes, int is_bf16,
               int two_shot, hipStream_t s,
               bf16_t* hb_pack = nullptr, int pack_cols = 0);
int car_pairs(void* state, int mode, const float* a, const int32_t* b, int idx_offset, long long n, int k,
              float* out_a, int32_t* out_b, hipStream_t s);
void car_set_gran_max(long long n);
int car_error(void* state);
const void* car_device(void* state);
long long car_max_bytes(void* state);
int car_world(void* state);
int car_set_grid(void* state, int grid);
void car_destroy(void* state);
int decode_update(const int32_t* nxt, int32_t* finished, int32_t* sequences, int32_t* cur_len, int32_t* tokens,
                  int32_t* positions, int32_t* slot, int B, int L, int pad, int eos, hipStream_t s);
int cu_census(uint32_t* out, int blocks, hipStream_t s);
int cu_mask_stream_create(const uint32_t* mask, int words, hipStream_t* out);
int cu_mask_stream_get(hipStream_t s, uint32_t* mask, int words);
int stream_destroy(hipStream_t s);
int graph_kernel_nodes(hipGraph_t g);

}
```

### jax_llama_amd/csrc/kernels/norm_embed.hip

```cpp
#include "common.h"
#include "launchers.h"

namespace jla {

__global__ void __launch_bounds__(256) embedding_kernel(const int32_t* __restrict__ ids,
                                                        const bf16_t* __restrict__ table,
                                                        float* __restrict__ out, bf16_t* __restrict__ mirror,
                                                        int D, int V) {
  const int row = blockIdx.x;
  int id = ids[row];
  if ((id < 0 || id >= V) && threadIdx.x == 0) JLA_FLAG(JLA_BOUNDS_TOKEN);
  id = id < 0 ? 0 : (id >= V ? V - 1 : id);
  const u32x4* src = reinterpret_cast<const u32x4*>(table + (size_t)id * D);
  float4* dst = reinterpret_cast<float4*>(out + (size_t)row * D);
  u32x4* mdst = mirror ? reinterpret_cast<u32x4*>(mirror + (size_t)row * D) : nullptr;
  for (int i = threadIdx.x; i < D / 8; i += blockDim.x) {
    const u32x4 v = src[i];
    float f[8];
    unpack8(v, f);
    dst[2 * i] = make_float4(f[0], f[1], f[2], f[3]);
    dst[2 * i + 1] = make_float4(f[4], f[5], f[6], f[7]);
    if (mdst) mdst[i] = v;
  }
}

int embedding(const int32_t* ids, const bf16_t* table, float* out, bf16_t* mirror, int M, int D, int V,
              hipStream_t s) {
  if (D % 8) return -1;
  if (M == 0) return 0;
  embedding_kernel<<<M, 256, 0, s>>>(ids, table, out, mirror, D, V);
  JLA_CHECK_LAUNCH();
  return 0;
}

template <bool WEIGHTED>
__global__ void __launch_bounds__(256) rms_kernel(const float* __restrict__ x, const float* __restrict__ w,
                                                  void* __restrict__ out, int D, float eps) {
  __shared__ float red[16];
  const int row = blockIdx.x;
  const float4* xr = reinterpret_cast<const float4*>(x + (size_t)row * D);
  float ss = 0.f;
  for (int i = threadIdx.x; i < D / 4; i += blockDim.x) {
    float4 v = xr[i];
    ss += v.x * v.x + v.y * v.y + v.z * v.z + v.w * v.w;
  }
  ss = block_sum(ss, red);
  const float inv = rsqrtf(ss / (float)D + eps);
  if (WEIGHTED) {
    float4* o = reinterpret_cast<float4*>(static_cast<float*>(out) + (size_t)row * D);
    const float4* wr = reinterpret_cast<const float4*>(w);
    for (int i = threadIdx.x; i < D / 4; i += blockDim.x) {
      float4 v = xr[i], g = wr[i];
      o[i] = make_float4(v.x * inv * g.x, v.y * inv * g.y, v.z * inv * g.z, v.w * inv * g.w);
    }
  } else {
    uint2* o = reinterpret_cast<uint2*>(static_cast<bf16_t*>(out) + (size_t)row * D);
    for (int i = threadIdx.x; i < D / 4; i += blockDim.x) {
      float4 v = xr[i];
      o[i] = make_uint2(pack2bf(v.x * inv, v.y * inv), pack2bf(v.z * inv, v.w * inv));
    }
  }
}

int rms_scale(const float* x, bf16_t* out, int M, int D, float eps, hipStream_t s) {
  if (D % 4) return -1;
  if (M == 0) return 0;
  rms_kernel<false><<<M, 256, 0, s>>>(x, nullptr, out, D, eps);
  JLA_CHECK_LAUNCH();
  return 0;
}

__global__ void __launch_bounds__(256) rms_bf16_kernel(const bf16_t* __restrict__ x, bf16_t* __restrict__ out,
                                                       int D, float eps) {
  __shared__ float red[16];
  const int row = blockIdx.x;
  const u32x4* xr = reinterpret_cast<const u32x4*>(x + (size_t)row * D);
  u32x4* o = reinterpret_cast<u32x4*>(out + (size_t)row * D);
  float ss = 0.f;
  for (int i = threadIdx.x; i < D / 8; i += blockDim.x) {
    float f[8];
    unpack8(xr[i], f);
#pragma unroll
    for (int j = 0; j < 8; ++j) ss += f[j] * f[j];
  }
  ss = block_sum(ss, red);
  const float inv = rsqrtf(ss / (float)D + eps);
  for (int i = threadIdx.x; i < D / 8; i += blockDim.x) {
    float f[8];
    unpack8(xr[i], f);
#pragma unroll
    for (int j = 0; j < 8; ++j) f[j] *= inv;
    o[i] = pack8(f);
  }
}

__global__ void __launch_bounds__(256) rms_rowinv_kernel(const bf16_t* __restrict__ x, float* __restrict__ inv, int M,
                                                         int D, float eps) {
  const int row = blockIdx.x * 4 + (threadIdx.x >> 6), lane = threadIdx.x & 63;
  if (row >= M) return;
  const u32x4* xr = reinterpret_cast<const u32x4*>(x + (size_t)row * D);
  float s0 = 0.f, s1 = 0.f;
#pragma unroll 4
  for (int i = lane; i < D / 8; i += 64) {
    const u32x4 v = xr[i];
#pragma unroll
    for (int e = 0; e < 4; ++e) {
      const float lo = __uint_as_float(v[e] << 16), hi = __uint_as_float(v[e] & 0xffff0000u);
      s0 = fmaf(lo, lo, s0);
      s1 = fmaf(hi, hi, s1);
    }
  }
  const float t = wave_sum(s0 + s1);
  if (lane == 0) inv[row] = 1.f / sqrtf(t / (float)D + eps);
}

int rms_rowinv(const bf16_t* x, float* inv, int M, int D, float eps, hipStream_t s) {
  if (D % 8) return -1;
  if (M == 0) return 0;
  rms_rowinv_kernel<<<(M + 3) / 4, 256, 0, s>>>(x, inv, M, D, eps);
  JLA_CHECK_LAUNCH();
  return 0;
}

int rms_scale_bf16(const bf16_t* x, bf16_t* out, int M, int D, float eps, hipStream_t s) {
  if (D % 8) return -1;
  if (M == 0) return 0;
  rms_bf16_kernel<<<M, 256, 0, s>>>(x, out, D, eps);
  JLA_CHECK_LAUNCH();
  return 0;
}

int rmsnorm(const float* x, const float* w, float* out, int M, int D, float eps, hipStream_t s) {
  if (D % 4) return -1;
  if (M == 0) return 0;
  rms_kernel<true><<<M, 256, 0, s>>>(x, w, out, D, eps);
  JLA_CHECK_LAUNCH();
  return 0;
}

template <bool BF16>
__global__ void __launch_bounds__(256) residual_add_kernel(float* __restrict__ h, const void* __restrict__ p,
                                                           bf16_t* __restrict__ hb, long long n8) {
  for (long long i = (long long)blockIdx.x * blockDim.x + threadIdx.x; i < n8; i += (long long)gridDim.x * blockDim.x) {
    float a[8];
    if constexpr (BF16) {
      unpack8(reinterpret_cast<const u32x4*>(p)[i], a);
    } else {
      const float4 v0 = reinterpret_cast<const float4*>(p)[2 * i], v1 = reinterpret_cast<const float4*>(p)[2 * i + 1];
      a[0] = v0.x; a[1] = v0.y; a[2] = v0.z; a[3] = v0.w; a[4] = v1.x; a[5] = v1.y; a[6] = v1.z; a[7] = v1.w;
    }
    float4* hv = reinterpret_cast<float4*>(h) + 2 * i;
    float4 x0 = hv[0], x1 = hv[1];
    x0.x += a[0]; x0.y += a[1]; x0.z += a[2]; x0.w += a[3];
    x1.x += a[4]; x1.y += a[5]; x1.z += a[6]; x1.w += a[7];
    hv[0] = x0;
    hv[1] = x1;
    const float r[8] = {x0.x, x0.y, x0.z, x0.w, x1.x, x1.y, x1.z, x1.w};
    reinterpret_cast<u32x4*>(hb)[i] = pack8(r);
  }
}

int residual_add(float* h, const void* p, int p_bf16, bf16_t* hb, long long n, hipStream_t s) {
  if (n % 8) return -1;
  if (n == 0) return 0;
  const long long n8 = n / 8;
  const long long want = (n8 + 255) / 256;
  const int grid = (int)(want < 4096 ? want : 4096);
  if (p_bf16) residual_add_kernel<true><<<grid, 256, 0, s>>>(h, p, hb, n8);
  else residual_add_kernel<false><<<grid, 256, 0, s>>>(h, p, hb, n8);
  JLA_CHECK_LAUNCH();
  return 0;
}

__global__ void __launch_bounds__(256) prefetch_kernel(const u32x4* __restrict__ p, long long n16,
                                                       unsigned* __restrict__ sink, unsigned key) {
  constexpr int U = 16;
  unsigned acc = 0;
  const long long stride = (long long)gridDim.x * blockDim.x;
  long long i = (long long)blockIdx.x * blockDim.x + threadIdx.x;
  for (; i + (U - 1) * stride < n16; i += U * stride) {
    u32x4 v[U];
#pragma unroll
    for (int u = 0; u < U; ++u) v[u] = p[i + u * stride];
#pragma unroll
    for (int u = 0; u < U; ++u) acc ^= v[u][0] ^ v[u][3];
  }
  for (; i < n16; i += stride) acc ^= p[i][1];
  if (acc == key) sink[0] = acc;
}

int prefetch(const void* p, long long nbytes, int grid, unsigned* sink, hipStream_t s) {
  if (nbytes <= 0) return 0;
  prefetch_kernel<<<grid, 256, 0, s>>>(static_cast<const u32x4*>(p), nbytes / 16, sink, 0x9e3779b9u);
  JLA_CHECK_LAUNCH();
  return 0;
}
// ... 58 lines not shown
```

### jax_llama_amd/models/llama.py

```python
from __future__ import annotations

from dataclasses import dataclass
from typing import Any, Dict, List, Optional, Tuple

import numpy as np
import torch

from .. import ops
from ..config import LLaMAConfig
from ..ops import reference as ref
from ..parallel.comm import NO_COMM, TPComm
from ..parallel.partition import shard_tree
from .kv_cache import KVCache
from .modules import LLaMABlockCollection
from .weights import Fp8Linear, PackedLinear

BF16 = torch.bfloat16


def _t(x) -> torch.Tensor:
    if torch.is_tensor(x):
        return x
    return torch.as_tensor(np.asarray(x))


@dataclass
class CausalLMOutput:

    logits: Optional[torch.Tensor] = None
    past_key_values: Optional[KVCache] = None
    hidden_states: Optional[Tuple[torch.Tensor, ...]] = None
    attentions: Optional[Tuple[torch.Tensor, ...]] = None

    def __getitem__(self, k):
        if isinstance(k, int):
            return self.to_tuple()[k]
        return getattr(self, k)

    def __setitem__(self, k, v):
        setattr(self, k, v)

    def to_tuple(self):
        return tuple(v for v in (self.logits, self.past_key_values, self.hidden_states, self.attentions)
                     if v is not None)


@dataclass
class ScoreOutput:

    token_logprobs: torch.Tensor
    is_greedy: torch.Tensor
    mask: torch.Tensor

    def __getitem__(self, k):
        if isinstance(k, int):
            return (self.token_logprobs, self.is_greedy, self.mask)[k]
        return getattr(self, k)


@dataclass
class BaseModelOutput:
    last_hidden_state: torch.Tensor = None
    hidden_states: Optional[Tuple[torch.Tensor, ...]] = None
    attentions: Optional[Tuple[torch.Tensor, ...]] = None

    def __getitem__(self, k):
        if isinstance(k, int):
            return tuple(v for v in (self.last_hidden_state, self.hidden_states, self.attentions)
                         if v is not None)[k]
        return getattr(self, k)


class LayerWeights:
    __slots__ = ("qkv", "o", "gu", "down", "attention_norm", "ffn_norm")

    def __init__(self):
        for s in self.__slots__:
            setattr(self, s, None)


def mask_to_kv_start(mask: torch.Tensor, device) -> Tuple[torch.Tensor, Optional[torch.Tensor]]:
    m = mask.detach().to("cpu").to(torch.int64)
    b, t = m.shape
    valid = m != 0
    first = torch.where(valid.any(1), valid.to(torch.int8).argmax(1), torch.full((b,), t, dtype=torch.int64))
    after = torch.arange(t)[None, :] >= first[:, None]
    if bool((after & ~valid).any()):
        return torch.zeros(b, dtype=torch.int32, device=device), m.to(torch.uint8).to(device).contiguous()
    return first.to(torch.int32).to(device), None


_DTYPE_NAMES = {"float32": torch.float32, "fp32": torch.float32, "f32": torch.float32,
                "bfloat16": BF16, "bf16": BF16}


def _resolve_dtype(d, default):
    if d is None:
# ... 122 lines not shown
        nqkv = (self.n_heads + 2 * self.n_kv_heads) * hd
        for lw in self.layers:
            lw.attention_norm = torch.ones(d, dtype=torch.float32, device=dev)
            lw.ffn_norm = torch.ones(d, dtype=torch.float32, device=dev)
            lw.qkv = PackedLinear.random(nqkv, d, dev, std, gen)
            lw.o = PackedLinear.random(d, self.n_heads * hd, dev, std, gen)
            lw.gu = PackedLinear.random(2 * self.ffn, d, dev, std, gen)
            lw.down = PackedLinear.random(d, self.ffn, dev, std, gen)
        self.lm_head = PackedLinear.random(self.vocab_local, d, dev, std, gen)
        self.lm_head_f32 = self.lm_head.dense().float().contiguous() if self.precision == "highest" else None
        return self

    def init_weights(self, rng=None, input_shape: Optional[Tuple[int, ...]] = None, params: Optional[Dict] = None,
                     std: Optional[float] = None) -> Dict:
        from ..parallel.partition import flatten_tree, unflatten_tree
        from ..utils.checkpoint import meta_state_dict_to_params, random_meta_state_dict
        if rng is None:
            seed = self.seed
        elif isinstance(rng, torch.Generator):
            seed = int(rng.initial_seed())
        else:
            seed = int(np.asarray(rng).reshape(-1)[-1])
        c = self.config
        sd = random_meta_state_dict(c, seed=seed, std=c.initializer_range if std is None else std,
                                    dtype=torch.float32, norm_jitter=0.0)
        rand = meta_state_dict_to_params(sd, c.num_hidden_layers)
        if c.tie_word_embeddings:
            rand.pop("lm_head", None)
        if params is None:
            return rand
        flat_r, flat_p = flatten_tree(rand), flatten_tree(params)
        missing = set(self._missing_keys) | (set(flat_r) - set(flat_p))
        for k in missing:
            flat_p[k] = flat_r[k]
        self._missing_keys = set()
        return unflatten_tree(flat_p)

    def save_pretrained(self, save_directory: str) -> str:
        from ..utils.native_ckpt import save_pretrained
        return save_pretrained(self, save_directory)

    @classmethod
    def from_pretrained(cls, directory: str, device="cpu", comm: Optional[TPComm] = None):
        from ..utils.native_ckpt import from_pretrained
        return from_pretrained(directory, device=device, comm=comm)

    WEIGHT_FORMATS = ("fp8_e4m3",)

    def quantize_weights_(self, fmt: str = "fp8_e4m3") -> "LLaMAForCausalLM":
        if fmt not in self.WEIGHT_FORMATS:
            raise ValueError(f"quantize_weights_: unknown format {fmt!r} (one of {self.WEIGHT_FORMATS})")
        if self.weight_format != "bf16":
            raise RuntimeError(f"quantize_weights_: the weights are already {self.weight_format}")
        if any(lw.qkv is None for lw in self.layers):
            raise RuntimeError("quantize_weights_: the model has no weights yet")
        for lw in self.layers:
            for name in ("qkv", "o", "gu", "down"):
                setattr(lw, name, Fp8Linear.from_linear(getattr(lw, name)))
        if self.device.type == "cuda":
            torch.cuda.empty_cache()
        return self

    @property
    def weight_format(self) -> str:
        return "fp8_e4m3" if any(getattr(lw.qkv, "fp8", False) for lw in self.layers) else "bf16"

    def weight_bytes(self) -> int:
        n = self.wte.numel() * 2 + self.lm_head.nbytes()
        for lw in self.layers:
            n += lw.qkv.nbytes() + lw.o.nbytes() + lw.gu.nbytes() + lw.down.nbytes()
        return n

    def streamed_weight_bytes_per_token(self) -> int:
        return self.weight_bytes() - self.wte.numel() * 2

    def init_cache(self, batch_size: int, max_length: int) -> KVCache:
        if max_length > self.rope_length:
            raise ValueError(f"max_length {max_length} exceeds the RoPE table ({self.rope_length}); "
                             "raise config.max_sequence_length")
        return KVCache(self.config.num_hidden_layers, batch_size, self.n_kv_heads, max_length,
                       self.head_dim, self.device)

    def _row_parallel(self, x: torch.Tensor, w: PackedLinear, h: torch.Tensor, hb: torch.Tensor,
                      x_packed: Optional[torch.Tensor] = None, mirror_packed: Optional[torch.Tensor] = None) -> None:
        if self.comm.size == 1:
            ops.linear_residual(x, w, h, mirror=hb, x_packed=x_packed, mirror_packed=mirror_packed)
        elif self.comm.linear_residual_(x, w, h, hb, x_packed=x_packed, hb_pack=mirror_packed):
            pass
        else:
            dt = self.comm.partial_dtype(x.numel() // x.shape[-1] * w.n, x.is_cuda)
            part = ops.linear(x, w, out_dtype=dt, x_packed=x_packed)
            self.comm.all_reduce_residual_(part, h, hb, hb_pack=mirror_packed, owned=True)

    def forward_tokens(self, ids: torch.Tensor, positions: torch.Tensor, cache: KVCache, slot0,
                       kv_start: torch.Tensor, key_mask: Optional[torch.Tensor] = None,
                       logits_mode: str = "last", collect_hidden: bool = False,
                       collect_attn: bool = False, targets: Optional[torch.Tensor] = None):
        if (logits_mode == "logprob") != (targets is not None):
            raise ValueError("logits_mode='logprob' takes `targets` (and no other mode does)")
        with ops.autotune.tp_scope(self.comm):
            return self._forward_tokens(ids, positions, cache, slot0, kv_start, key_mask, logits_mode,
                                        collect_hidden, collect_attn, targets)

    def _forward_tokens(self, ids, positions, cache, slot0, kv_start, key_mask, logits_mode, collect_hidden,
                        collect_attn, targets=None):
        b, s = ids.shape
        d = self.config.hidden_size
        hb = torch.empty(b * s, d, dtype=BF16, device=self.device)
        h = ops.embedding(ids.reshape(-1), self.wte, mirror=hb)
        hidden, attns = self.blocks(h, hb, positions, cache, slot0, kv_start, key_mask, s,
                                    output_hidden_states=collect_hidden, output_attentions=collect_attn)
        if logits_mode == "none":
            logits = None
        elif logits_mode == "logprob":
            off = self.tp_rank * self.vocab_local
            if self.precision == "highest":
                logits = ops.linear_f32_logprob(self.final_norm(h), self.lm_head_f32, targets, col_offset=off)
            else:
                logits = ops.linear_logprob(hb, self.lm_head, targets, rms_eps=self.eps, col_offset=off)
        elif self.precision == "highest":
            hl = h if logits_mode == "all" else h.reshape(b, s, d)[:, -1].contiguous()
            logits = ops.linear_f32(self.final_norm(hl), self.lm_head_f32)
            if logits_mode == "argmax":
                logits = ops.argmax(logits.contiguous())
        elif logits_mode == "argmax":
            logits = ops.linear_argmax(hb.reshape(b, s, d)[:, -1].contiguous(), self.lm_head, rms_eps=self.eps)
        else:
            hl = hb if logits_mode == "all" else hb.reshape(b, s, d)[:, -1].contiguous()
            logits = ops.linear(hl, self.lm_head, rms_eps=self.eps, out_dtype=torch.float32)
        return logits, h, hidden, attns

    def gather_logits(self, logits_local: torch.Tensor) -> torch.Tensor:
        if self.comm.size == 1:
            return logits_local
        g = self.comm.all_gather(logits_local)
        return g.permute(1, 0, 2).reshape(logits_local.shape[0], -1)

    def final_norm(self, h: torch.Tensor) -> torch.Tensor:
        return ops.rmsnorm(h, self.ln_f, self.eps)

    def _prepare_call(self, input_ids, attention_mask, position_ids, past_key_values):
        ids = _t(input_ids).to(self.device, torch.int32)
        b, s = ids.shape
        if position_ids is None:
            if past_key_values is not None:
                raise ValueError("Make sure to provide `position_ids` when passing `past_key_values`.")
            position_ids = torch.arange(s, dtype=torch.int32).expand(b, s)
        pos = _t(position_ids).to(self.device, torch.int32).reshape(b, s).contiguous()
        if past_key_values is None:
            cache = KVCache(self.config.num_hidden_layers, b, self.n_kv_heads, s, self.head_dim, self.device)
            slot0 = 0
        else:
            cache = past_key_values
            slot0 = cache.index
            if slot0 + s > cache.max_length:
                raise ValueError(f"cache overflow: {slot0}+{s} > {cache.max_length}")
        t_valid = slot0 + s
        if attention_mask is None:
            mask = torch.ones(b, t_valid, dtype=torch.int32)
        else:
            mask = _t(attention_mask).to("cpu").to(torch.int32)
            if mask.shape[1] >= t_valid:
                mask = mask[:, :t_valid]
            elif mask.shape[1] == s:
                mask = torch.cat([torch.ones(b, slot0, dtype=torch.int32), mask], 1)
            else:
                raise ValueError(f"attention_mask of shape {tuple(mask.shape)} does not cover {t_valid} slots")
        kv_start, key_mask = mask_to_kv_start(mask, self.device)
        return ids, pos, cache, slot0, kv_start, key_mask

    def __call__(self, input_ids, attention_mask=None, position_ids=None, params=None,
                 past_key_values: Optional[KVCache] = None, dropout_rng=None, train: bool = False,
                 output_attentions: Optional[bool] = None, output_hidden_states: Optional[bool] = None,
                 return_dict: Optional[bool] = None):
        if train:
            raise NotImplementedError("inference-only framework (reference dropout/remat paths are training-only)")
        if params is not None and id(params) != self._params_id:
            self.load_params(params)
        oa = self.config.output_attentions if output_attentions is None else output_attentions
        oh = self.config.output_hidden_states if output_hidden_states is None else output_hidden_states
        rd = self.config.return_dict if return_dict is None else return_dict
        ids, pos, cache, slot0, kv_start, key_mask = self._prepare_call(
            input_ids, attention_mask, position_ids, past_key_values)
        b, s = ids.shape
        logits, h, hidden, attns = self.forward_tokens(ids, pos, cache, slot0, kv_start, key_mask,
                                                       logits_mode="all", collect_hidden=oh,
                                                       collect_attn=oa)
        if past_key_values is not None:
            cache.advance(s)
        logits = self.gather_logits(logits).reshape(b, s, -1).to(self.dtype)
        hs = None
        if oh:
            hs = tuple(x.to(self.dtype) for x in hidden) + (self.final_norm(h).reshape(b, s, -1).to(self.dtype),)
        out = CausalLMOutput(logits=logits, past_key_values=past_key_values, hidden_states=hs,
                             attentions=tuple(attns) if oa else None)
        return out if rd else out.to_tuple()

    def score(self, input_ids, attention_mask=None, labels=None, ignore_index: int = -100) -> ScoreOutput:
        from ..runtime import engine as _engine
        ids = _t(input_ids).to("cpu", torch.int64)
        if ids.dim() != 2 or ids.shape[1] < 2:
            raise ValueError(f"score: input_ids must be (B, S) with S >= 2, got {tuple(ids.shape)}")
        b, s = ids.shape
        if s > self.rope_length:
            raise ValueError(f"score: {s} positions exceed the RoPE table ({self.rope_length}); "
                             "raise config.max_sequence_length")
        lab = ids if labels is None else _t(labels).to("cpu", torch.int64)
        if lab.shape != ids.shape:
            raise ValueError(f"score: labels {tuple(lab.shape)} must have input_ids' shape {tuple(ids.shape)}")
        if attention_mask is None:
            mask = torch.ones(b, s, dtype=torch.int32)
        else:
# ... 83 lines not shown
```

### jax_llama_amd/models/modules.py

```python
from __future__ import annotations

from typing import List, Optional

import torch

from .. import ops
from ..ops import reference as ref


class LLaMAAttention:
    def __init__(self, model, layer_idx: int):
        self.model = model
        self.layer_idx = layer_idx

    @property
    def weights(self):
        return self.model.layers[self.layer_idx]

    def __call__(self, h, hb, positions, cache, slot0, kv_start, key_mask, seq_len: int,
                 output_attentions: bool = False, pk: Optional["PackedActs"] = None) -> Optional[torch.Tensor]:
        m, lw = self.model, self.weights
        kc, vc = cache.layer(self.layer_idx)
        splits = og = 0
        o_state = None
        if not output_attentions:
            og = ops.qkv_attention_o_groups(hb, lw.o, m.n_heads, m.n_kv_heads) if seq_len == 1 else 0
            o_state = m.comm.fused_o_state(hb, lw.o) if og else None
            og = og if o_state is not None else 0
            splits = ops.qkv_attention_splits(hb, lw.qkv, kc, seq_len, m.n_heads, m.n_kv_heads, key_mask, og)
            if og and not splits:
                og = 0
                splits = ops.qkv_attention_splits(hb, lw.qkv, kc, seq_len, m.n_heads, m.n_kv_heads, key_mask)
        if splits:
            hb_p = pk.hb if pk else None
            o = (lw.o, h, hb, hb_p, o_state) if og else None
            att_p = pk.att if pk is not None and not og else None
            a = ops.linear_qkv_attention(hb, lw.qkv, m.eps, m.rope, positions, kc, vc, slot0, kv_start, m.n_heads,
                                         m.n_kv_heads, m.head_dim, splits, x_packed=pk.hb_in() if pk else None,
                                         out_packed=att_p, o=o)
            if not og:
                m._row_parallel(a, lw.o, h, hb, x_packed=att_p, mirror_packed=hb_p)
            if pk is not None and pk.hb is not None:
                pk.hb_ok = True
            return None
        q = ops.linear_qkv_rope(hb, lw.qkv, m.eps, m.rope, positions, kc, vc, slot0, seq_len,
                                m.n_heads, m.n_kv_heads, m.head_dim, x_packed=pk.hb_in() if pk else None)
        b = hb.shape[0] // seq_len
        q4 = q.reshape(b, seq_len, m.n_heads, m.head_dim)
        weights = None
        att_p = None
        if output_attentions:
            s0 = int(slot0) if not torch.is_tensor(slot0) else int(slot0.item())
            _, weights = ref.attention(q4, kc, vc, s0, kv_start, key_mask, return_weights=True)
            a = ops.attention(q4, kc, vc, slot0, kv_start, key_mask)
        else:
            att_p = pk.att if pk is not None and ops.attention_packs(q4, kc, key_mask) else None
            a = ops.attention(q4, kc, vc, slot0, kv_start, key_mask, out_packed=att_p)
        m._row_parallel(a, lw.o, h, hb, x_packed=att_p, mirror_packed=pk.hb if pk else None)
        if pk is not None and pk.hb is not None:
            pk.hb_ok = True
        return weights


class LLaMAMLP:
    def __init__(self, model, layer_idx: int):
        self.model = model
        self.layer_idx = layer_idx

    def __call__(self, h, hb, pk: Optional["PackedActs"] = None) -> None:
        m, lw = self.model, self.model.layers[self.layer_idx]
        g = ops.linear_swiglu(hb, lw.gu, rms_eps=m.eps, x_packed=pk.hb_in() if pk else None,
                              out_packed=pk.act if pk else None)

        m._row_parallel(g, lw.down, h, hb, x_packed=pk.act if pk else None, mirror_packed=pk.hb if pk else None)


class LLaMABlock:

    def __init__(self, model, layer_idx: int):
        self.attention = LLaMAAttention(model, layer_idx)
        self.feed_forward = LLaMAMLP(model, layer_idx)

    def __call__(self, h, hb, positions, cache, slot0, kv_start, key_mask, seq_len: int,
                 output_attentions: bool = False, pk: Optional["PackedActs"] = None):
        w = self.attention(h, hb, positions, cache, slot0, kv_start, key_mask, seq_len, output_attentions, pk)
        self.feed_forward(h, hb, pk)
        return w


class PackedActs:

    def __init__(self, rows: int, model, device, full: bool = True):
        self.hb = ops.packed_empty(rows, model.config.hidden_size, device) if full else None
        self.att = ops.packed_empty(rows, model.n_heads * model.head_dim, device)
        self.act = ops.packed_empty(rows, model.ffn, device) if full else None
        self.hb_ok = False

    def hb_in(self) -> Optional[torch.Tensor]:
        return self.hb if self.hb_ok else None


class LLaMABlockCollection:

    def __init__(self, model):
        self.blocks: List[LLaMABlock] = [LLaMABlock(model, i) for i in range(len(model.layers))]
        self.model = model

    def __len__(self):
        return len(self.blocks)

    def __call__(self, h, hb, positions, cache, slot0, kv_start, key_mask, seq_len: int,
                 output_hidden_states: bool = False, output_attentions: bool = False):
        hidden, attns = [], []
        b = hb.shape[0] // seq_len
        rows = hb.shape[0]
        pk = None
        if (ops.PACKED_X and hb.is_cuda and ops.PACKED_X_MIN_M <= rows <= min(ops.PACKED_ATT_MAX_M, ops.SKINNY_M)
                and self.model.comm.packs_residual(rows * self.model.config.hidden_size * 4)):
            pk = PackedActs(rows, self.model, hb.device, full=rows <= ops.PACKED_X_MAX_M)
        for blk in self.blocks:
            if output_hidden_states:
                hidden.append(h.reshape(b, seq_len, -1).clone())
            w = blk(h, hb, positions, cache, slot0, kv_start, key_mask, seq_len, output_attentions, pk)
            if output_attentions:
                attns.append(w)
        return hidden, attns
```

### jax_llama_amd/ops/__init__.py

```python
from __future__ import annotations

import contextlib
import os
from typing import Optional

import torch

from . import autotune
from . import reference as ref
from ._ext import available as ext_available
from ._ext import ext

BF16 = torch.bfloat16

MODE_STORE = 0
MODE_RESIDUAL = 1
MODE_SWIGLU = 2
MODE_QKV = 3

GEMV_VARIANT = int(os.environ.get("JLA_GEMV_VARIANT", "0"))


def _is_gpu(t: torch.Tensor) -> bool:
    return t.device.type == "cuda"
# ... 44 lines not shown
    if not _is_gpu(table):
        out = ref.embedding(ids, table)
        if mirror is not None:
            mirror.copy_(out.to(BF16))
        return out
    out = torch.empty(ids.numel(), table.shape[1], dtype=torch.float32, device=table.device)
    ext().embedding(ids.reshape(-1).to(torch.int32), table, out, mirror)
    return out


def rms_scale(x: torch.Tensor, eps: float) -> torch.Tensor:
    if not _is_gpu(x):
        return ref.rms_scale(x, eps)
    out = torch.empty(x.shape, dtype=BF16, device=x.device)
    ext().rms_scale(x, out, float(eps))
    return out


def residual_add_(h: torch.Tensor, p: torch.Tensor, mirror: Optional[torch.Tensor] = None) -> torch.Tensor:
    if not _is_gpu(h):
        h.add_(p.float().view_as(h))
        if mirror is not None:
            mirror.copy_(h.to(BF16))
        return h
    assert h.is_contiguous() and h.dtype == torch.float32
    if mirror is None or h.numel() % 8:
        h.add_(p.view_as(h))
        if mirror is not None:
            mirror.copy_(h)
        return h
    ext().residual_add(h, p.contiguous(), mirror)
    return h


PREFETCH_GRID = int(os.environ.get("JLA_PREFETCH_GRID", "128"))


def prefetch(t: torch.Tensor) -> None:
    if _is_gpu(t):
        ext().prefetch(t, PREFETCH_GRID)


def linear_f32(x: torch.Tensor, w: torch.Tensor) -> torch.Tensor:
    if not _is_gpu(x):
        return x.float() @ w.float().t()
    y = torch.empty(x.shape[0], w.shape[0], dtype=torch.float32, device=x.device)
    ext().gemm_f32(x.float().contiguous(), w.float().contiguous(), y)
    return y


def rmsnorm(x: torch.Tensor, weight: torch.Tensor, eps: float) -> torch.Tensor:
    if not _is_gpu(x):
        return ref.rmsnorm(x, weight, eps)
    out = torch.empty(x.shape, dtype=torch.float32, device=x.device)
    ext().rmsnorm(x.float().contiguous(), weight.float().contiguous(), out, float(eps))
    return out


BOUNDS_CODES = {0: "token id outside the vocabulary", 1: "KV-cache write past the cache (slot >= T)",
                2: "decode step past the sequence buffer", 3: "attention asked for keys past the cache",
                4: "position outside the RoPE table"}


class BoundsError(RuntimeError):
    pass


def bounds_error(reset: bool = False) -> int:
    if not ext_available():
        return 0
    return int(ext().bounds_error(bool(reset)))


def check_bounds(reset: bool = True):
    if not ext_available() or not getattr(ext(), "DEBUG_BOUNDS", False):
        return
    err = bounds_error(reset)
    if err:
        raise BoundsError("device-side index out of range: " +
                          "; ".join(v for k, v in BOUNDS_CODES.items() if err >> k & 1))


def linear(x: torch.Tensor, w, rms_eps: Optional[float] = None, out_dtype=BF16,
           out: Optional[torch.Tensor] = None, x_packed: Optional[torch.Tensor] = None) -> torch.Tensor:
    if not _is_gpu(x):
        r = ref.linear(x, w.dense(), rms_eps, out_dtype)
        if out is not None:
            out.copy_(r)
            return out
        return r
    m = x.shape[0]
    if out is None:
        out = torch.empty(m, w.n, dtype=out_dtype, device=x.device)
    _gpu_linear(x, w, out, MODE_STORE, rms_eps, True, None, x_packed)
    return out


def linear_residual(x: torch.Tensor, w, residual: torch.Tensor, rms_eps: Optional[float] = None,
                    accumulate: bool = True, mirror: Optional[torch.Tensor] = None,
                    x_packed: Optional[torch.Tensor] = None, mirror_packed: Optional[torch.Tensor] = None) -> torch.Tensor:
    if not _is_gpu(x):
        ref.linear_residual(x, w.dense(), residual, rms_eps, accumulate)
        if mirror is not None:
            mirror.copy_(residual.to(BF16))
        return residual
    _gpu_linear(x, w, residual, MODE_RESIDUAL, rms_eps, accumulate, mirror, x_packed, mirror_packed)
    return residual


def linear_swiglu(x: torch.Tensor, w, rms_eps: Optional[float] = None, x_packed: Optional[torch.Tensor] = None,
                  out_packed: Optional[torch.Tensor] = None) -> torch.Tensor:
    if not _is_gpu(x):
        return ref.linear_swiglu(x, w.dense(), rms_eps)
    out = torch.empty(x.shape[0], w.n // 2, dtype=BF16, device=x.device)
    _gpu_linear(x, w, out, MODE_SWIGLU, rms_eps, True, None, x_packed, out_packed)
    return out


PACKED_X = os.environ.get("JLA_PACKED_X", "1") != "0"
PACKED_X_MIN_M = int(os.environ.get("JLA_PACKED_X_MIN_M", "9"))
PACKED_X_MAX_M = int(os.environ.get("JLA_PACKED_X_MAX_M", "64"))
PACKED_ATT_MAX_M = int(os.environ.get("JLA_PACKED_ATT_MAX_M", "64"))
SKINNY_M = 64
XP_VARIANTS, SPLIT_VARIANTS = autotune.XP_VARIANTS, autotune.SPLIT_VARIANTS


def packed_rows(m: int) -> int:
    return 16 if m <= 16 else (32 if m <= 32 else 64)


def packed_empty(m: int, cols: int, device) -> torch.Tensor:
    return torch.empty(packed_rows(m), cols, dtype=BF16, device=device)


class _Dequantized:

    def __init__(self, weight, n, k):
        self.weight, self.n, self.k = weight, n, k


def is_fp8(w) -> bool:
    return bool(getattr(w, "fp8", False))


def bf16_weight(w):
    if not is_fp8(w):
        return w
    buf = workspace.get(f"w8_deq_{w.n}x{w.k}", w.n * w.k, BF16, w.device).view(w.n // 16, w.k // 32, 64, 8)
    ext().dequant_fp8(w.qweight, w.scale, w.n, w.k, buf)
    return _Dequantized(buf, w.n, w.k)


def _w8_fast(e, x, w, mode) -> bool:
    return x.shape[0] > 0 and e.gemv_w8_plan_check(x.shape[0], w.n, w.k, mode, x.dtype != BF16)[0] == 0


def _gpu_linear(x, w, out, mode, rms_eps, accumulate, mirror=None, x_packed=None, pack_out=None):
    assert x.is_contiguous() and out.is_contiguous()
    assert x.shape[1] == w.k, (x.shape, w.k)
    m = x.shape[0]
    e = ext()
    if is_fp8(w):
        if _w8_fast(e, x, w, mode):
            e.linear_skinny_w8(x, w.qweight, w.scale, w.n, w.k, out, mode, -1.0 if rms_eps is None else float(rms_eps),
                               bool(accumulate), mirror, pack_out if mode != MODE_STORE else None)
            return
        w = bf16_weight(w)
    if m > e.SKINNY_MAX_M:
        x_packed = pack_out = None
    v = TILED if m > e.SKINNY_MAX_M else _variant(e, x, w, mode, x_packed, pack_out)
    if v == TILED and pack_out is not None and not _tiled_packs(e, m, w.n, w.k, x.device, mode, rms_eps):
        v = 1
    if v == TILED:
        _tiled(e, x, w.weight, w.n, w.k, out, mode, rms_eps, accumulate, mirror, pack_out)
    else:
        ws, tk = _skinny_ws(e, m, w.n, w.k, mode, x.device)
        e.linear_skinny(x, w.weight, w.n, w.k, out, mode, -1.0 if rms_eps is None else float(rms_eps),
                        bool(accumulate), v, ws, tk, mirror, x_packed if v in XP_VARIANTS else None, pack_out)


def linear_tp_residual(x: torch.Tensor, w, h: torch.Tensor, hb: torch.Tensor, state: int,
                       x_packed: Optional[torch.Tensor] = None, hb_pack: Optional[torch.Tensor] = None) -> torch.Tensor:
    e = ext()
    m = x.shape[0]
    assert x.dtype == BF16 and x.is_contiguous() and m <= e.SKINNY_MAX_M, (x.dtype, x.shape)
    v = _variant(e, x, w, MODE_RESIDUAL, x_packed, pack_out=True)
    if v not in autotune.GEMV_VARIANTS:
        v = 1
    ws = tk = None
    if v in SPLIT_VARIANTS:
        ws, tk = _skinny_ws(e, m, w.n, w.k, MODE_RESIDUAL, x.device)
    e.linear_tp_residual(state, x, w.weight, w.n, w.k, h, hb, v, x_packed if v in XP_VARIANTS else None, hb_pack,
                         ws, tk)
    return h


def tiled_tp_residual(x: torch.Tensor, w, h: torch.Tensor, hb: torch.Tensor, state: int) -> bool:
    e = ext()
    m = x.shape[0]
    assert x.dtype == BF16 and x.is_contiguous(), (x.dtype, x.shape)
    ks, tm = autotune.choose_gemm_plan(e, m, w.n, w.k, x.device, MODE_STORE, False)
    if tm not in autotune.G5_TILES and ks <= 1:
        return False
    ks, tm, ws = _gemm_ws(e, m, w.n, w.k, x.device, MODE_STORE, False)
    e.gemm_tp_residual(state, x, w.weight, w.n, w.k, h, hb, ks, ws, tm)
    return True


TILED = autotune.TILED_VARIANT
QKV_DIRECT = os.environ.get("JLA_QKV_DIRECT", "1") != "0"


def _fused_rms(e, mode, rms_eps) -> bool:
    return rms_eps is not None and mode != MODE_RESIDUAL


def _tiled_input(x, rms_eps, fused=False):
    if rms_eps is not None and not fused:
        return rms_scale(x, rms_eps)
    return x if x.dtype == BF16 else x.to(BF16)


def _gemm_ws(e, m, n, k, device, mode=MODE_STORE, rms=False):
    ks, tm = autotune.choose_gemm_plan(e, m, n, k, device, mode, rms)
    if tm in autotune.G5_TILES:
        eks = e.gemm5_ksplit(k, ks)
        return ks, tm, workspace.get("gemm_ws", eks * m * (n + 1), torch.float32, device)
    ws = workspace.get("gemm_ws", ks * m * (n + 1), torch.float32, device) if ks > 1 else None
    return ks, tm, ws


def _rms_ws(x, fused: bool, ks: int):
    if not fused or ks > 1:
        return None
    return workspace.get("gemm_rms", x.shape[0], torch.float32, x.device)


def _tiled(e, x, weight, n, k, out, mode, rms_eps, accumulate, mirror=None, pack_out=None):
    fused = _fused_rms(e, mode, rms_eps)
    xb = _tiled_input(x, rms_eps, fused)
    ks, tm, ws = _gemm_ws(e, x.shape[0], n, k, x.device, mode, fused)
    e.gemm(xb, weight, n, k, out, mode, bool(accumulate), mirror, ks, ws, float(rms_eps) if fused else -1.0, tm,
           pack_out, _rms_ws(x, fused, ks))


def _tiled_packs(e, m, n, k, device, mode, rms_eps) -> bool:
    if e is None or m > SKINNY_M or mode not in (MODE_RESIDUAL, MODE_SWIGLU):
        return False
    ks, tm = autotune.choose_gemm_plan(e, m, n, k, device, mode, _fused_rms(e, mode, rms_eps))
    if tm in autotune.G5_TILES:
        return True
    return ks > 1


def _variant(e, x, w, mode, x_packed=None, pack_out=None, no_split=False) -> int:
    xp_in, p_out = x_packed is not None, pack_out is not None
    if GEMV_VARIANT:
        v = GEMV_VARIANT
        xp, split = autotune.GEMV_VARIANTS.get(v, (False, False))
        if (xp and not xp_in) or (p_out and v == TILED and not _tiled_packs(
                e, x.shape[0], w.n, w.k, x.device, mode, None if mode == MODE_RESIDUAL else 1e-5)) or (
                split and (no_split or x.dtype != BF16 or w.n // 16 > autotune.SPLIT_MAX_GROUPS)):
            v = 1
        if v == 12 and mode == MODE_SWIGLU:
            v = 15
        return v
    m = x.shape[0]
    pmode = MODE_STORE if mode == MODE_QKV else mode
    ws, tk = _skinny_ws(e, m, w.n, w.k, pmode, x.device)
    ncols = w.n // 2 if pmode == MODE_SWIGLU else w.n
    odt = torch.float32 if pmode == MODE_RESIDUAL else BF16
    scratch = workspace.get("tune_out", m * ncols, odt, x.device).view(m, ncols)
    mirror = workspace.get("tune_mirror", m * ncols, BF16, x.device).view(m, ncols) if (
        p_out and pmode == MODE_RESIDUAL) else None
    pscratch = workspace.get("tune_pack", packed_rows(m) * ncols, BF16, x.device).view(-1, ncols) if p_out else None

    tiled_packs = p_out and _tiled_packs(e, m, w.n, w.k, x.device, pmode, None if pmode == MODE_RESIDUAL else 1e-5)

    def run(v, xx, wt):
        if v == TILED:
            _tiled(e, xx, wt, w.n, w.k, scratch, pmode, None if pmode == MODE_RESIDUAL else 1e-5, True, mirror,
                   pscratch if tiled_packs else None)
        else:
            e.linear_skinny(xx, wt, w.n, w.k, scratch, pmode, 1e-5, True, v, ws, tk, mirror,
                            x_packed if v in XP_VARIANTS else None, pscratch)

    return autotune.choose(e, x, w, pmode, run, xp_in=xp_in, pack_out=p_out, no_split=no_split,
                           tiled_packs=tiled_packs)


_SK_SIZES = {}


def _skinny_ws(e, m, n, k, mode, device):
    key = (m, n, k, mode)
    sz = _SK_SIZES.get(key)
    if sz is None:
        sz = _SK_SIZES[key] = tuple(e.skinny_workspace(m, n))
    floats, tickets = sz
    return (workspace.get("skinny", max(1, floats), torch.float32, device),
            workspace.get_zeroed("skinny_tickets", max(1, tickets), torch.int32, device))


def rope_kv_write(qkv: torch.Tensor, table: torch.Tensor, positions: torch.Tensor,
                  k_cache: torch.Tensor, v_cache: torch.Tensor, slot0, seq_len: int,
                  n_heads: int, n_kv_heads: int, head_dim: int) -> torch.Tensor:
    if not _is_gpu(qkv):
        s0 = int(slot0) if not torch.is_tensor(slot0) else int(slot0.item())
        return ref.rope_kv_write(qkv, table, positions, k_cache, v_cache, s0, seq_len,
                                 n_heads, n_kv_heads, head_dim)
    m = qkv.shape[0]
    q = torch.empty(m, n_heads, head_dim, dtype=BF16, device=qkv.device)
    slot_t = _slot_tensor(slot0, qkv.device)
    ext().rope_kv_write(qkv, table, positions.reshape(-1).to(torch.int32), k_cache, v_cache,
                        slot_t, int(seq_len), int(n_heads), int(n_kv_heads), int(head_dim), q)
    return q


def linear_qkv_rope(x: torch.Tensor, w, rms_eps: Optional[float], table: torch.Tensor, positions: torch.Tensor,
                    k_cache: torch.Tensor, v_cache: torch.Tensor, slot0, seq_len: int, n_heads: int,
                    n_kv_heads: int, head_dim: int, x_packed: Optional[torch.Tensor] = None) -> torch.Tensor:
    if not _is_gpu(x):
        s0 = int(slot0) if not torch.is_tensor(slot0) else int(slot0.item())
        return ref.linear_qkv_rope(x, w.dense(), rms_eps, table, positions, k_cache, v_cache, s0, seq_len,
                                   n_heads, n_kv_heads, head_dim)
    m = x.shape[0]
    e = ext()
    if is_fp8(w):
        if _w8_fast(e, x, w, MODE_QKV):
            q = torch.empty(m, n_heads, head_dim, dtype=BF16, device=x.device)
            e.linear_qkv_w8(x, w.qweight, w.scale, w.n, w.k, -1.0 if rms_eps is None else float(rms_eps), table,
                            positions.reshape(-1).to(torch.int32), k_cache, v_cache, _slot_tensor(slot0, x.device),
                            int(seq_len), int(n_heads), int(n_kv_heads), int(head_dim), q)
            return q
        w = bf16_weight(w)
    if m > e.SKINNY_MAX_M:
        x_packed = None
    v = TILED if m > e.SKINNY_MAX_M else _variant(e, x, w, MODE_QKV, x_packed)
    if v == TILED:
        ks, tm, ws = _gemm_ws(e, m, w.n, w.k, x.device, MODE_STORE, _fused_rms(e, MODE_QKV, rms_eps))
        fused = _fused_rms(e, MODE_QKV, rms_eps)
        if ks == 1 and fused and QKV_DIRECT and e.gemm_qkv_direct_ok(m, tm, w.k):
            q = torch.empty(m, n_heads, head_dim, dtype=BF16, device=x.device)
            e.gemm_qkv(_tiled_input(x, rms_eps, fused), w.weight, w.n, w.k, table, positions.reshape(-1).to(torch.int32),
                       k_cache, v_cache, _slot_tensor(slot0, x.device), int(seq_len), int(n_heads), int(n_kv_heads),
                       int(head_dim), q, 1, None, float(rms_eps), tm, _rms_ws(x, fused, 1))
            return q
        if ks == 1:
            qkv = linear(x, w, rms_eps=rms_eps)
            return rope_kv_write(qkv, table, positions, k_cache, v_cache, slot0, seq_len, n_heads, n_kv_heads,
                                 head_dim)
        q = torch.empty(m, n_heads, head_dim, dtype=BF16, device=x.device)
        e.gemm_qkv(_tiled_input(x, rms_eps, fused), w.weight, w.n, w.k, table, positions.reshape(-1).to(torch.int32),
                   k_cache, v_cache, _slot_tensor(slot0, x.device), int(seq_len), int(n_heads), int(n_kv_heads),
                   int(head_dim), q, ks, ws, float(rms_eps) if fused else -1.0, tm)
        return q
    q = torch.empty(m, n_heads, head_dim, dtype=BF16, device=x.device)
    ws, tk = _skinny_ws(e, m, w.n, w.k, MODE_QKV, x.device)
    e.linear_qkv(x, w.weight, w.n, w.k, -1.0 if rms_eps is None else float(rms_eps), table,
                 positions.reshape(-1).to(torch.int32), k_cache, v_cache, _slot_tensor(slot0, x.device),
                 int(seq_len), int(n_heads), int(n_kv_heads), int(head_dim), q, v, ws, tk,
                 x_packed if v in XP_VARIANTS else None)
    return q


QKV_ATTN = int(os.environ.get("JLA_QKV_ATTN", "1"))
QKV_ATTN_SPL = int(os.environ.get("JLA_QKV_ATTN_SPL", "2"))
QKV_ATTN_O = int(os.environ.get("JLA_QKV_ATTN_O", "0"))
_CUS = {}


class InLaunchTimeout(RuntimeError):
    """An in-launch wait gave up (the fused qkv + attention launch: a qkv workgroup never published)."""


def check_inlaunch() -> None:
    global QKV_ATTN
    for (name, _dev, _dt), buf in list(workspace._bufs.items()):
        if name.startswith("zeroed:") and name.endswith("qa_sync") and buf.is_cuda and int(buf[2].item()):
            QKV_ATTN = 0
            buf.zero_()
            workspace.generation += 1
            raise InLaunchTimeout("fused qkv + attention launch: a wait timed out (the attention workgroups on the qkv "
                                  "workgroups, or the o workgroups on the attention ones; error word qa_sync[2]); the "
                                  "fused path is now off for this process")


def _num_cus(device) -> int:
    key = str(device)
    if key not in _CUS:
        _CUS[key] = torch.cuda.get_device_properties(device).multi_processor_count
    return _CUS[key]


def qkv_attention_o_groups(x: torch.Tensor, w_o, n_heads: int, n_kv_heads: int) -> int:
    if not QKV_ATTN_O or not _is_gpu(x) or is_fp8(w_o):
        return 0
    return int(ext().qkv_attn_o_groups(x.shape[0], n_heads // n_kv_heads, w_o.n, w_o.k))


def qkv_attention_splits(x: torch.Tensor, w, k_cache: torch.Tensor, seq_len: int, n_heads: int, n_kv_heads: int,
                         key_mask: Optional[torch.Tensor] = None, o_groups: int = 0) -> int:
    if not QKV_ATTN or seq_len != 1 or key_mask is not None or not _is_gpu(x) or x.dtype != BF16 or is_fp8(w):
        return 0
    m = x.shape[0]
    if QKV_ATTN == 1 and (m > 4 or n_heads < 8 * n_kv_heads):
        return 0
    return int(ext().qkv_attn_splits(m, m, n_kv_heads, n_heads // n_kv_heads, k_cache.shape[2], w.n,
                                     _num_cus(x.device), 1, int(o_groups)))


def _qkv_attention_spl(e, m, w, k_cache, n_heads, n_kv_heads, device, o_groups=0) -> int:
    if QKV_ATTN_SPL > 1 and e.qkv_attn_splits(m, m, n_kv_heads, n_heads // n_kv_heads, k_cache.shape[2], w.n,
                                               _num_cus(device), 2, int(o_groups)) > 0:
        return 2
    return 1


def linear_qkv_attention(x: torch.Tensor, w, rms_eps: Optional[float], table: torch.Tensor, positions: torch.Tensor,
                         k_cache: torch.Tensor, v_cache: torch.Tensor, slot0, kv_start: torch.Tensor, n_heads: int,
                         n_kv_heads: int, head_dim: int, splits: int, x_packed: Optional[torch.Tensor] = None,
                         out_packed: Optional[torch.Tensor] = None, spl: Optional[int] = None,
                         o: Optional[tuple] = None) -> torch.Tensor:
    e = ext()
    m = x.shape[0]
    dev = x.device
    rep = n_heads // n_kv_heads
    q = workspace.get("qa_q", m * n_heads * head_dim, BF16, dev).view(m, n_heads, head_dim)
    out = torch.empty(m, n_heads * head_dim, dtype=BF16, device=dev)
    ws = workspace.get("qa_ws", m * n_kv_heads * splits * rep * (head_dim + 4), torch.float32, dev)
    tickets = workspace.get_zeroed("qa_tickets", max(m * n_kv_heads, 64), torch.int32, dev)
    sync = workspace.get_zeroed("qa_sync", int(e.qkv_attn_sync_ints()), torch.int32, dev)
    og = 0 if o is None else int(e.qkv_attn_o_groups(m, rep, o[0].n, o[0].k))
    spl = _qkv_attention_spl(e, m, w, k_cache, n_heads, n_kv_heads, dev, og) if spl is None else int(spl)
    sk_ws = sk_tk = None
    if spl > 1:
        sk_ws, sk_tk = _skinny_ws(e, m, w.n, w.k, MODE_QKV, dev)
    ow = oh = ohb = ohp = None
    on = ok = 0
    tp_state = 0
    if o is not None:
        wo, oh, ohb, ohp, tp_state = o
        ow, on, ok = wo.weight, wo.n, wo.k
    e.linear_qkv_attn(x, w.weight, w.n, w.k, -1.0 if rms_eps is None else float(rms_eps), table,
                      positions.reshape(-1).to(torch.int32), k_cache, v_cache, _slot_tensor(slot0, dev), n_heads,
                      n_kv_heads, head_dim, q, kv_start, out, out_packed, ws, tickets, sync, k_cache.shape[2], splits,
                      x_packed, spl, sk_ws, sk_tk, ow, on, ok, oh, ohb, ohp, int(tp_state or 0))
    return out


def attention_packs(q: torch.Tensor, k_cache: torch.Tensor, key_mask: Optional[torch.Tensor] = None) -> bool:
    bsz, s, h, dh = q.shape
    if s != 1:
        return False
    rc, _why, _kernel, _nsplit, packs, *_ = ext().attn_decode_plan_check(
        bsz, h, k_cache.shape[1], dh, k_cache.shape[2], key_mask is not None)
    return rc == 0 and bool(packs)


def attention(q: torch.Tensor, k_cache: torch.Tensor, v_cache: torch.Tensor, slot0, kv_start: torch.Tensor,
              key_mask: Optional[torch.Tensor] = None, max_kv: Optional[int] = None,
              out_packed: Optional[torch.Tensor] = None) -> torch.Tensor:
    bsz, s, h, dh = q.shape
    if not _is_gpu(q):
        s0 = int(slot0) if not torch.is_tensor(slot0) else int(slot0.item())
        return ref.attention(q, k_cache, v_cache, s0, kv_start, key_mask).reshape(bsz * s, h * dh)
    out = torch.empty(bsz * s, h * dh, dtype=BF16, device=q.device)
    slot_t = _slot_tensor(slot0, q.device)
    t_cap = int(max_kv) if max_kv is not None else k_cache.shape[2]
    e = ext()
    if s == 1:
        hkv = k_cache.shape[1]
        _rc, _why, _kernel, nsplit, _packs, ws_floats, n_tickets, *_ = e.attn_decode_plan_check(
            bsz, h, hkv, dh, t_cap, key_mask is not None)
        ws = workspace.get("attn_decode", ws_floats, torch.float32, q.device)
        tickets = workspace.get_zeroed("attn_tickets", n_tickets, torch.int32, q.device)
        e.attn_decode(q, k_cache, v_cache, slot_t, kv_start, key_mask, out, ws, tickets, t_cap, nsplit, out_packed)
    else:
        e.attn_prefill(q, k_cache, v_cache, slot_t, kv_start, key_mask, out)
    return out


def _slot_tensor(slot0, device):
    if torch.is_tensor(slot0):
        return slot0
    t = torch.tensor([int(slot0)], dtype=torch.int32, device=device)
    return t


def argmax(logits: torch.Tensor):
    if not _is_gpu(logits):
        v, i = logits.float().max(-1)
        return ref.argmax(logits), v
    b = logits.shape[0]
    idx = torch.empty(b, dtype=torch.int32, device=logits.device)
    val = torch.empty(b, dtype=torch.float32, device=logits.device)
    ext().argmax(logits, idx, val)
    return idx, val


ARGMAX_FUSED_MIN_M = 256
SKINNY_ARGMAX = os.environ.get("JLA_SKINNY_ARGMAX", "1") != "0"


def linear_argmax(x: torch.Tensor, w, rms_eps: Optional[float] = None):
    m = x.shape[0]
    if not _is_gpu(x):
        return argmax(linear(x, w, rms_eps, out_dtype=torch.float32))
    w = bf16_weight(w)
    if m <= ext().SKINNY_MAX_M and SKINNY_ARGMAX:
        e = ext()
        v = _variant(e, x, w, MODE_STORE, no_split=True)
        if v in autotune.ROW_MAJOR_VARIANTS and v != 10:
            part = workspace.get("skinny_argmax", m * (w.n // 16) * 2, torch.float32, x.device)
            idx = torch.empty(m, dtype=torch.int32, device=x.device)
            val = torch.empty(m, dtype=torch.float32, device=x.device)
            e.linear_skinny_argmax(x, w.weight, w.n, w.k, -1.0 if rms_eps is None else float(rms_eps), v, part, idx,
                                   val)
            return idx, val
    if m < ARGMAX_FUSED_MIN_M:
        return argmax(linear(x, w, rms_eps, out_dtype=torch.float32))
    e = ext()
    assert x.is_contiguous() and x.shape[1] == w.k, (x.shape, w.k)
    xb = x if x.dtype == BF16 else x.to(BF16)
    ws = workspace.get("gemm_argmax", e.gemm_argmax_workspace(m, w.n), torch.float32, x.device)
    idx = torch.empty(m, dtype=torch.int32, device=x.device)
    val = torch.empty(m, dtype=torch.float32, device=x.device)
    e.gemm_argmax(xb, w.weight, w.n, w.k, ws, -1.0 if rms_eps is None else float(rms_eps), idx, val,
                  _rms_ws(x, rms_eps is not None, 1))
    return idx, val


MODE_LOGPROB = 10
LOGPROB_CHUNK_BYTES = 256 << 20


def logprob(logits: torch.Tensor, targets: torch.Tensor, col_offset: int = 0):
    if not _is_gpu(logits):
        return ref.logprob(logits, targets, col_offset)
    assert logits.dim() == 2 and logits.dtype == torch.float32 and logits.is_contiguous(), (logits.shape, logits.dtype)
    m = logits.shape[0]
    out = torch.empty(3, m, dtype=torch.float32, device=logits.device)
    ext().logprob_rows(logits, targets.reshape(-1).to(torch.int32), int(col_offset), out[0], out[1], out[2])
    return out[0], out[1], out[2]


def logprob_fused(x: torch.Tensor, w, rms_eps: Optional[float] = None) -> bool:
    if not _is_gpu(x) or x.shape[0] < ARGMAX_FUSED_MIN_M:
        return False
    rms = rms_eps is not None
    return ext().gemm_plan_check(x.shape[0], w.n, w.k, MODE_LOGPROB, rms, 1, 0, rms) == 0


def _logprob_chunks(m: int, n: int):
    rows = max(1, LOGPROB_CHUNK_BYTES // (4 * n))
    return [(r0, min(m, r0 + rows)) for r0 in range(0, m, rows)]


def linear_logprob(x: torch.Tensor, w, targets: torch.Tensor, rms_eps: Optional[float] = None, col_offset: int = 0):
    if not _is_gpu(x):
        return ref.linear_logprob(x, w.dense(), targets, rms_eps, col_offset)
    w = bf16_weight(w)
    m = x.shape[0]
    assert x.is_contiguous() and x.shape[1] == w.k, (x.shape, w.k)
    tg = targets.reshape(-1).to(torch.int32)
    assert tg.numel() == m, (tg.shape, m)
    out = torch.empty(3, m, dtype=torch.float32, device=x.device)
    if logprob_fused(x, w, rms_eps):
        e = ext()
        xb = x if x.dtype == BF16 else x.to(BF16)
        ws = workspace.get("gemm_logprob", e.gemm_logprob_workspace(m, w.n), torch.float32, x.device)
        e.gemm_logprob(xb, w.weight, w.n, w.k, ws, -1.0 if rms_eps is None else float(rms_eps), tg, int(col_offset),
                       out[0], out[1], out[2], _rms_ws(x, rms_eps is not None, 1))
    else:
        for r0, r1 in _logprob_chunks(m, w.n):
            logits = linear(x[r0:r1], w, rms_eps, out_dtype=torch.float32)
            ext().logprob_rows(logits, tg[r0:r1], int(col_offset), out[0, r0:r1], out[1, r0:r1], out[2, r0:r1])
    return out[0], out[1], out[2]


def linear_f32_logprob(x: torch.Tensor, w: torch.Tensor, targets: torch.Tensor, col_offset: int = 0):
    m = x.shape[0]
    tg = targets.reshape(-1).to(torch.int32)
    parts = [logprob(linear_f32(x[r0:r1], w), tg[r0:r1], col_offset) for r0, r1 in _logprob_chunks(m, w.shape[0])]
    return tuple(torch.cat([p[i] for p in parts]) for i in range(3))


def logprob_combine(tgt: torch.Tensor, mx: torch.Tensor, se: torch.Tensor):
    if tgt.dim() == 1:
        tgt, mx, se = tgt[None], mx[None], se[None]
    tgt, mx, se = tgt.float(), mx.float(), se.float()
    big = mx.max(0).values
    safe = torch.where(torch.isinf(big), torch.zeros_like(big), big)
    total = torch.zeros_like(big)
    t = torch.zeros_like(big)
    for r in range(mx.shape[0]):
        total = total + se[r] * torch.exp(mx[r] - safe)
        t = t + tgt[r]
    lse = big + torch.log(total)
    return t - lse, lse, t == big


SAMPLER_MAX_K = 64


def topk_candidates(logits: torch.Tensor, k: int, idx_offset: int = 0):
    if not _is_gpu(logits):
        v, i = ref.topk_sorted(logits, k)
        return v, i + idx_offset
    e = ext()
    b, v = logits.shape
    c = e.topk_chunks(v) * k
# ... 35 lines not shown
```

Before: 42820 tokens/s.

## Fuse RMS row statistic into split-K residual reduce and reuse it downstream

The split-K reduce kernel for residual GEMMs now also accumulates the sum of squares of the bf16 mirror row and writes the inverse RMS per row into a stat buffer. The following fused-norm GEMMs (QKV, SwiGLU/store, argmax) can mark the statistic as ready and skip the separate rms_rowinv pass that re-reads the activations. This saves one launch and one full read of the hidden state per norm. The cost is Python-side state tracking to keep the stat valid and a per-row wave reduction inside the reduce kernel.

```diff
diff --git a/jax_llama_amd/csrc/bindings.cpp b/jax_llama_amd/csrc/bindings.cpp
--- a/jax_llama_amd/csrc/bindings.cpp
+++ b/jax_llama_amd/csrc/bindings.cpp
@@ -417,9 +417,10 @@
   return ptr<float>(*rws);
 }
 
-void gemm(Tensor x, Tensor w, int64_t n, int64_t k, Tensor out, int64_t mode, bool accumulate,
+bool gemm(Tensor x, Tensor w, int64_t n, int64_t k, Tensor out, int64_t mode, bool accumulate,
           c10::optional<Tensor> mirror, int64_t ksplit, c10::optional<Tensor> ws, double rms_eps, int64_t tile,
-          c10::optional<Tensor> pack_out, c10::optional<Tensor> rms_ws, int64_t n_body) {
+          c10::optional<Tensor> pack_out, c10::optional<Tensor> rms_ws, int64_t n_body,
+          c10::optional<Tensor> stat_out, double stat_eps, bool stat_ready) {
   check_gpu(x, "x");
   check_packed(w, n, k);
   check(n_body >= 0 && (n_body == 0 || jla::gemm_tail_width((int)tile) > 0), "gemm n_body: tail-balanced tiles only");
@@ -438,16 +439,36 @@
   const bool slabs = check_gemm_ws(ws, k, ksplit, m, n, rms_eps >= 0, tile);
   size_t rfl = 0;
   float* rws = rms_ws_ptr(rms_ws, m, &rfl);
+  jla::RowStat st;
+  st.ready = stat_ready;
+  check(!stat_ready || rws, "gemm stat_ready: the statistic lives in rms_ws");
+  if (stat_out.has_value()) {
+    check(mode == 1 && mir, "gemm stat_out: residual mode with its mirror");
+    check_gpu(*stat_out, "stat_out");
+    check(stat_out->scalar_type() == torch::kFloat32 && stat_out->numel() >= m, "stat_out: fp32, >= M floats");
+    st.out = ptr<float>(*stat_out);
+    st.eps = (float)stat_eps;
+  }
   gemm_rc(jla::gemm(cbf(x), w.data_ptr(), out.data_ptr(), m, n, k, mode, accumulate,
                     out.scalar_type() == torch::kFloat32, mir, pqa.pack ? &pqa : nullptr,
                     slabs ? ptr<float>(*ws) : nullptr, slabs ? ws->numel() : 0, ksplit, stream(), (float)rms_eps,
-                    (int)tile, rws, rfl, (int)n_body),
+                    (int)tile, rws, rfl, (int)n_body, &st),
           "gemm");
+  return st.written;
+}
+
+void rms_rowinv(Tensor x, Tensor inv, double eps) {
+  check_gpu(x, "x");
+  check_gpu(inv, "inv");
+  check(x.dim() == 2 && x.scalar_type() == torch::kBFloat16, "rms_rowinv: x must be bf16 [M, D]");
+  check(inv.scalar_type() == torch::kFloat32 && inv.numel() >= x.size(0), "rms_rowinv: inv fp32, >= M floats");
+  rc(jla::rms_rowinv(cbf(x), ptr<float>(inv), x.size(0), x.size(1), (float)eps, stream()), "rms_rowinv");
 }
 
 void gemm_qkv(Tensor x, Tensor w, int64_t n, int64_t k, Tensor table, Tensor positions, Tensor kc, Tensor vc,
               Tensor slot, int64_t seq_len, int64_t h, int64_t hkv, int64_t dh, Tensor q, int64_t ksplit,
-              c10::optional<Tensor> ws, double rms_eps, int64_t tile, c10::optional<Tensor> rms_ws) {
+              c10::optional<Tensor> ws, double rms_eps, int64_t tile, c10::optional<Tensor> rms_ws,
+              bool stat_ready) {
   check_gpu(x, "x");
   check_packed(w, n, k);
   check(x.dim() == 2 && x.size(1) == k && x.scalar_type() == torch::kBFloat16, "x must be bf16 [M, K]");
@@ -456,9 +477,12 @@
   const bool slabs = check_gemm_ws(ws, k, ksplit, m, n, rms_eps >= 0, tile);
   size_t rfl = 0;
   float* rws = rms_ws_ptr(rms_ws, m, &rfl);
+  jla::RowStat st;
+  st.ready = stat_ready;
+  check(!stat_ready || rws, "gemm_qkv stat_ready: the statistic lives in rms_ws");
   gemm_rc(jla::gemm(cbf(x), w.data_ptr(), nullptr, m, n, k, MODE_QKV, 0, 0, nullptr, &qa,
                     slabs ? ptr<float>(*ws) : nullptr, slabs ? ws->numel() : 0, ksplit, stream(), (float)rms_eps,
-                    (int)tile, rws, rfl),
+                    (int)tile, rws, rfl, 0, &st),
           "gemm_qkv");
 }
 
@@ -550,7 +574,7 @@
 }
 
 void gemm_argmax(Tensor x, Tensor w, int64_t n, int64_t k, Tensor ws, double rms_eps, Tensor idx, Tensor val,
-                 c10::optional<Tensor> rms_ws) {
+                 c10::optional<Tensor> rms_ws, bool stat_ready) {
   check_gpu(x, "x");
   check_packed(w, n, k);
   check(x.dim() == 2 && x.size(1) == k && x.scalar_type() == torch::kBFloat16, "x must be bf16 [M, K]");
@@ -565,8 +589,9 @@
         "gemm_argmax outputs");
   size_t rfl = 0;
   float* rws = rms_ws_ptr(rms_ws, m, &rfl);
+  check(!stat_ready || rws, "gemm_argmax stat_ready: the statistic lives in rms_ws");
   rc(jla::gemm_argmax(cbf(x), w.data_ptr(), ptr<float>(ws), ws.numel(), m, n, k, (float)rms_eps, ptr<int32_t>(idx),
-                      ptr<float>(val), stream(), rws, rfl),
+                      ptr<float>(val), stream(), rws, rfl, stat_ready),
      "gemm_argmax");
 }
 
@@ -823,7 +848,9 @@
   m.def("gemm", &gemm, py::arg("x"), py::arg("w"), py::arg("n"), py::arg("k"), py::arg("out"), py::arg("mode"),
         py::arg("accumulate"), py::arg("mirror") = py::none(), py::arg("ksplit") = 1, py::arg("ws") = py::none(),
         py::arg("rms_eps") = -1.0, py::arg("tile") = 0, py::arg("pack_out") = py::none(),
-        py::arg("rms_ws") = py::none(), py::arg("n_body") = 0);
+        py::arg("rms_ws") = py::none(), py::arg("n_body") = 0, py::arg("stat_out") = py::none(),
+        py::arg("stat_eps") = 0.0, py::arg("stat_ready") = false);
+  m.def("rms_rowinv", &rms_rowinv, py::arg("x"), py::arg("inv"), py::arg("eps"));
   m.def("gemm_tail_split", [](int64_t tiles_m, int64_t n, int64_t width, int64_t cus) {
     const int nb = jla::gemm_tail_split((int)tiles_m, (int)n, (int)width, cus > 0 ? (int)cus : jla::gemm_num_cus());
     return std::make_pair((int64_t)nb, nb > 0 ? (n - nb * width + 127) / 128 : (int64_t)0);
@@ -831,6 +858,11 @@
   m.def("gemm_plan_check", [](int64_t m, int64_t n, int64_t k, int64_t mode, bool rms, int64_t ksplit, int64_t tile,
                               bool has_rms_ws, int64_t n_body) {
     return jla::gemm_plan_check((int)m, (int)n, (int)k, (int)mode, rms, (int)ksplit, (int)tile, has_rms_ws, (int)n_body);
+  }, py::arg("m"), py::arg("n"), py::arg("k"), py::arg("mode"), py::arg("rms"), py::arg("ksplit"), py::arg("tile"),
+     py::arg("has_rms_ws"), py::arg("n_body") = 0);
+  m.def("gemm_plan_norm", [](int64_t m, int64_t n, int64_t k, int64_t mode, bool rms, int64_t ksplit, int64_t tile,
+                             bool has_rms_ws, int64_t n_body) {
+    return jla::gemm_plan_norm((int)m, (int)n, (int)k, (int)mode, rms, (int)ksplit, (int)tile, has_rms_ws, (int)n_body);
   }, py::arg("m"), py::arg("n"), py::arg("k"), py::arg("mode"), py::arg("rms"), py::arg("ksplit"), py::arg("tile"),
      py::arg("has_rms_ws"), py::arg("n_body") = 0);
   m.def("gemv_plan_check", [](int64_t m, int64_t n, int64_t k, int64_t mode, bool x_f32, bool x_packed,
@@ -865,9 +897,10 @@
   m.def("gemm_qkv", &gemm_qkv, py::arg("x"), py::arg("w"), py::arg("n"), py::arg("k"), py::arg("table"),
         py::arg("positions"), py::arg("kc"), py::arg("vc"), py::arg("slot"), py::arg("seq_len"), py::arg("h"),
         py::arg("hkv"), py::arg("dh"), py::arg("q"), py::arg("ksplit"), py::arg("ws"), py::arg("rms_eps") = -1.0,
-        py::arg("tile") = 0, py::arg("rms_ws") = py::none());
+        py::arg("tile") = 0, py::arg("rms_ws") = py::none(), py::arg("stat_ready") = false);
   m.def("gemm_argmax", &gemm_argmax, py::arg("x"), py::arg("w"), py::arg("n"), py::arg("k"), py::arg("ws"),
-        py::arg("rms_eps"), py::arg("idx"), py::arg("val"), py::arg("rms_ws") = py::none());
+        py::arg("rms_eps"), py::arg("idx"), py::arg("val"), py::arg("rms_ws") = py::none(),
+        py::arg("stat_ready") = false);
   m.def("gemm_argmax_workspace", [](int64_t m, int64_t n) { return (int64_t)jla::gemm_argmax_workspace_floats(m, n); });
   m.def("gemm_logprob", &gemm_logprob, py::arg("x"), py::arg("w"), py::arg("n"), py::arg("k"), py::arg("ws"),
         py::arg("rms_eps"), py::arg("targets"), py::arg("col_offset"), py::arg("tgt"), py::arg("mx"), py::arg("se"),
diff --git a/jax_llama_amd/csrc/kernels/common.h b/jax_llama_amd/csrc/kernels/common.h
--- a/jax_llama_amd/csrc/kernels/common.h
+++ b/jax_llama_amd/csrc/kernels/common.h
@@ -114,6 +114,19 @@
   return v;
 }
 
+JLA_DEV void rms_piece_acc(const u32x4 v, float& s0, float& s1) {
+#pragma unroll
+  for (int e = 0; e < 4; ++e) {
+    const float lo = __uint_as_float(v[e] << 16), hi = __uint_as_float(v[e] & 0xffff0000u);
+    s0 = fmaf(lo, lo, s0);
+    s1 = fmaf(hi, hi, s1);
+  }
+}
+JLA_DEV float rms_row_inv(float s0, float s1, int D, float eps) {
+  const float t = wave_sum(s0 + s1);
+  return 1.f / sqrtf(t / (float)D + eps);
+}
+
 JLA_DEV float block_sum(float v, float* red) {
   const int lane = threadIdx.x & 63, wid = threadIdx.x >> 6, nw = (blockDim.x + 63) >> 6;
   v = wave_sum(v);
diff --git a/jax_llama_amd/csrc/kernels/gemm.hip b/jax_llama_amd/csrc/kernels/gemm.hip
--- a/jax_llama_amd/csrc/kernels/gemm.hip
+++ b/jax_llama_amd/csrc/kernels/gemm.hip
@@ -1072,6 +1072,60 @@
   }
 }
 
+template <int KS, int CH>
+__global__ void __launch_bounds__(256)
+    gemm_reduce_stat_kernel(const float* __restrict__ ws, int ksplit, float* __restrict__ h, int M, int N,
+                            int accumulate, bf16_t* __restrict__ mirror, bf16_t* __restrict__ pack,
+                            float* __restrict__ stat, float eps) {
+  const int row = blockIdx.x * 4 + (threadIdx.x >> 6), lane = threadIdx.x & 63;
+  if (row >= M) return;
+  const int ks = KS ? KS : ksplit, np = N >> 3;
+  const size_t slab4 = (size_t)M * N / 4, row4 = (size_t)row * (N >> 2);
+  float4* const hr = reinterpret_cast<float4*>(h) + row4;
+  float s0 = 0.f, s1 = 0.f;
+  for (int p0 = lane; p0 < np; p0 += 64 * CH) {
+    float4 hv[CH][2], v[CH][2];
+#pragma unroll
+    for (int c = 0; c < CH; ++c) {
+      const int p = min(p0 + 64 * c, np - 1);
+      hv[c][0] = hr[2 * p];
+      hv[c][1] = hr[2 * p + 1];
+    }
+#pragma unroll
+    for (int c = 0; c < CH; ++c) {
+      const int p = min(p0 + 64 * c, np - 1);
+      v[c][0] = sum_splits(ws, ks, slab4, row4 + 2 * p);
+      v[c][1] = sum_splits(ws, ks, slab4, row4 + 2 * p + 1);
+    }
+#pragma unroll
+    for (int c = 0; c < CH; ++c) {
+      const int p = p0 + 64 * c;
+      if (p >= np) continue;
+      float4 r[2];
+#pragma unroll
+      for (int u = 0; u < 2; ++u) {
+        r[u] = hv[c][u];
+        if (accumulate) {
+          r[u].x += v[c][u].x;
+          r[u].y += v[c][u].y;
+          r[u].z += v[c][u].z;
+          r[u].w += v[c][u].w;
+        } else {
+          r[u] = v[c][u];
+        }
+        hr[2 * p + u] = r[u];
+      }
+      const u32x4 pk = {pack2bf(r[0].x, r[0].y), pack2bf(r[0].z, r[0].w), pack2bf(r[1].x, r[1].y),
+                        pack2bf(r[1].z, r[1].w)};
+      *reinterpret_cast<u32x4*>(mirror + (size_t)row * N + 8 * p) = pk;
+      if (pack) *reinterpret_cast<u32x4*>(pack + pack_off(row, 8 * p, N)) = pk;
+      rms_piece_acc(pk, s0, s1);
+    }
+  }
+  const float inv = rms_row_inv(s0, s1, N, eps);
+  if (lane == 0) stat[row] = inv;
+}
+
 constexpr int TPR_ELEMS = 4096;
 static_assert(TPR_ELEMS / 2 * 8 == TPRES_REGION, "one fused-exchange region per workgroup");
 __global__ void __launch_bounds__(256)
@@ -1182,6 +1236,11 @@
 int gemm_plan_check(int M, int N, int K, int mode, int rms, int ksplit, int tile, int has_rms_ws, int n_body) {
   return gemm_plan(M, N, K, mode, rms != 0, ksplit, tile, has_rms_ws != 0, n_body, num_cus(), g_g4_default).rc;
 }
+int gemm_plan_norm(int M, int N, int K, int mode, int rms, int ksplit, int tile, int has_rms_ws, int n_body) {
+  const GemmPlanResult r =
+      gemm_plan(M, N, K, mode, rms != 0, ksplit, tile, has_rms_ws != 0, n_body, num_cus(), g_g4_default);
+  return r.rc != 0 ? r.rc : (int)r.plan.norm;
+}
 
 struct GemmArgs {
   const bf16_t* x;
@@ -1194,11 +1253,12 @@
   float* rms_ws;
   QKVArgs qa;
   hipStream_t s;
+  bool stat_ready = false;
 };
 
 static bool g4_row_stat(const GemmArgs& a, const GemmPlan& p, const float*& inv) {
   inv = p.norm == NORM_PRECOMPUTED ? a.rms_ws : nullptr;
-  return inv == nullptr || rms_rowinv(a.x, a.rms_ws, a.M, a.K, a.rms_eps, a.s) == 0;
+  return inv == nullptr || a.stat_ready || rms_rowinv(a.x, a.rms_ws, a.M, a.K, a.rms_eps, a.s) == 0;
 }
 
 static int g_g4_group = 0;
@@ -1372,12 +1432,29 @@
 
 static int launch_reduce(const float* ws, int ksplit, void* out, int M, int N, int K, int mode, int accumulate,
                          int out_f32, bf16_t* mirror, const QKVArgs* qkv, const float* ssq, float rms_eps,
-                         hipStream_t s) {
+                         hipStream_t s, RowStat* stat = nullptr) {
   const size_t total4 = (size_t)M * N / (mode == MODE_SWIGLU ? 8 : 4);
   const int rgrid = (int)((total4 + 255) / 256);
   QKVArgs qa{};
   if (qkv) qa = *qkv;
   const float eps = ssq ? rms_eps : 0.f;
+  if (mode == MODE_RESIDUAL && stat && stat->out && mirror && (N & 7) == 0) {
+#define JLA_RSTAT(KS, CH)                                                                                      \
+  gemm_reduce_stat_kernel<KS, CH><<<(M + 3) / 4, 256, 0, s>>>(ws, ksplit, static_cast<float*>(out), M, N, accumulate, \
+                                                              mirror, qa.pack, stat->out, stat->eps)
+    if (ksplit == 2)
+      JLA_RSTAT(2, 8);
+    else if (ksplit == 3)
+      JLA_RSTAT(3, 4);
+    else if (ksplit == 4)
+      JLA_RSTAT(4, 4);
+    else
+      JLA_RSTAT(0, 2);
+#undef JLA_RSTAT
+    JLA_CHECK_LAUNCH();
+    stat->written = true;
+    return 0;
+  }
   switch (mode) {
     case MODE_STORE:
       gemm_reduce_kernel<MODE_STORE><<<rgrid, 256, 0, s>>>(ws, ksplit, out, M, N, accumulate, out_f32, nullptr, qa,
@@ -1408,7 +1485,8 @@
 
 int gemm(const bf16_t* x, const void* W, void* out, int M, int N, int K, int mode, int accumulate, int out_f32,
          bf16_t* mirror, const QKVArgs* qkv, float* ws, size_t ws_floats, int ksplit, hipStream_t s,
-         float rms_eps, int tile, float* rms_ws, size_t rms_ws_floats, int n_body) {
+         float rms_eps, int tile, float* rms_ws, size_t rms_ws_floats, int n_body, RowStat* stat) {
+  if (stat) stat->written = false;
   const bool has_rms_ws = rms_ws != nullptr && rms_ws_floats >= (size_t)M;
   const GemmPlanResult r =
       gemm_plan(M, N, K, mode, rms_eps >= 0.f, ksplit, tile, has_rms_ws, n_body, num_cus(), g_g4_default);
@@ -1418,6 +1496,7 @@
   const u32x4* w = static_cast<const u32x4*>(W);
   if (!p.reduce) {
     GemmArgs a{x, w, out, M, N, K, accumulate, out_f32, nullptr, rms_eps, nullptr, rms_ws, QKVArgs{}, s};
+    a.stat_ready = stat && stat->ready;
     switch (mode) {
       case MODE_QKV:
         a.out = nullptr, a.accumulate = a.out_f32 = 0, a.qa = *qkv;
@@ -1442,7 +1521,7 @@
   float* ssq = p.norm != NORM_NONE ? ws + slabs : nullptr;
   launch_plan<MODE_PARTIAL>(GemmArgs{x, w, ws, M, N, K, 0, 1, nullptr, rms_eps, ssq, nullptr, QKVArgs{}, s}, p);
   JLA_CHECK_LAUNCH();
-  return launch_reduce(ws, p.ksplit, out, M, N, K, mode, accumulate, out_f32, mirror, qkv, ssq, rms_eps, s);
+  return launch_reduce(ws, p.ksplit, out, M, N, K, mode, accumulate, out_f32, mirror, qkv, ssq, rms_eps, s, stat);
 }
 
 JLA_DEV void amax_merge(float& bv, int& bi, float ov, int oi) {
@@ -1513,14 +1592,14 @@
 size_t gemm_argmax_workspace_floats(int M, int N) { return (size_t)M * ((N + G2_BN - 1) / G2_BN) * 4 * 2; }
 
 int gemm_argmax(const bf16_t* x, const void* W, float* ws, size_t ws_floats, int M, int N, int K, float rms_eps,
-                int32_t* idx, float* val, hipStream_t s, float* rms_ws, size_t rms_ws_floats) {
+                int32_t* idx, float* val, hipStream_t s, float* rms_ws, size_t rms_ws_floats, bool stat_ready) {
   const bool has_rms_ws = rms_ws != nullptr && rms_ws_floats >= (size_t)M;
   const GemmPlanResult r = gemm_plan(M, N, K, MODE_ARGMAX, rms_eps >= 0.f, 1, 0, has_rms_ws, 0, 0, g_g4_default);
   if (r.rc != 0 || r.plan.family == GEMM_NONE) return r.rc;
   if (ws == nullptr || ws_floats < gemm_argmax_workspace_floats(M, N)) return -3;
-  launch_plan<MODE_ARGMAX>(
-      GemmArgs{x, static_cast<const u32x4*>(W), ws, M, N, K, 0, 1, nullptr, rms_eps, nullptr, rms_ws, QKVArgs{}, s},
-      r.plan);
+  GemmArgs a{x, static_cast<const u32x4*>(W), ws, M, N, K, 0, 1, nullptr, rms_eps, nullptr, rms_ws, QKVArgs{}, s};
+  a.stat_ready = stat_ready;
+  launch_plan<MODE_ARGMAX>(a, r.plan);
   JLA_CHECK_LAUNCH();
   const int P = (N + G2_BN - 1) / G2_BN * (r.plan.family == GEMM4 ? 2 : 4);
   launch_argmax_partials(reinterpret_cast<const float2*>(ws), P, M, idx, val, s);
diff --git a/jax_llama_amd/csrc/kernels/launchers.h b/jax_llama_amd/csrc/kernels/launchers.h
--- a/jax_llama_amd/csrc/kernels/launchers.h
+++ b/jax_llama_amd/csrc/kernels/launchers.h
@@ -67,10 +67,18 @@
 int linear_skinny_w8(const void* x, int x_is_f32, const void* W8, const float* scale, void* out, int M, int N, int K,
                      int mode, float rms_eps, int accumulate, int out_f32, const QKVArgs* qkv, hipStream_t s);
 int clock_probe(int iters, int grid, unsigned long long* out, hipStream_t s);
+struct RowStat {
+  float* out = nullptr;
+  float eps = 0.f;
+  bool ready = false;
+  bool written = false;
+};
 int gemm(const bf16_t* x, const void* W, void* out, int M, int N, int K, int mode, int accumulate, int out_f32,
          bf16_t* mirror, const QKVArgs* qkv, float* ws, size_t ws_floats, int ksplit, hipStream_t s,
-         float rms_eps = -1.f, int tile = 0, float* rms_ws = nullptr, size_t rms_ws_floats = 0, int n_body = 0);
+         float rms_eps = -1.f, int tile = 0, float* rms_ws = nullptr, size_t rms_ws_floats = 0, int n_body = 0,
+         RowStat* stat = nullptr);
 int gemm_plan_check(int M, int N, int K, int mode, int rms, int ksplit, int tile, int has_rms_ws, int n_body);
+int gemm_plan_norm(int M, int N, int K, int mode, int rms, int ksplit, int tile, int has_rms_ws, int n_body);
 int gemm_ksplit(int M, int N, int K);
 size_t gemm_workspace_floats(int M, int N, int K);
 int gemm_tp_groups(int M, int N);
@@ -80,7 +88,8 @@
 void gemm_set_g4_group(int gm);
 void gemm5_set_diag(int d);
 int gemm_argmax(const bf16_t* x, const void* W, float* ws, size_t ws_floats, int M, int N, int K, float rms_eps,
-                int32_t* idx, float* val, hipStream_t s, float* rms_ws = nullptr, size_t rms_ws_floats = 0);
+                int32_t* idx, float* val, hipStream_t s, float* rms_ws = nullptr, size_t rms_ws_floats = 0,
+                bool stat_ready = false);
 size_t gemm_argmax_workspace_floats(int M, int N);
 int argmax_partials(const float* part, int P, int M, int32_t* idx, float* val, hipStream_t s);
 int gemm_logprob(const bf16_t* x, const void* W, float* ws, size_t ws_floats, int M, int N, int K, float rms_eps,
diff --git a/jax_llama_amd/csrc/kernels/norm_embed.hip b/jax_llama_amd/csrc/kernels/norm_embed.hip
--- a/jax_llama_amd/csrc/kernels/norm_embed.hip
+++ b/jax_llama_amd/csrc/kernels/norm_embed.hip
@@ -102,16 +102,10 @@
   float s0 = 0.f, s1 = 0.f;
 #pragma unroll 4
   for (int i = lane; i < D / 8; i += 64) {
-    const u32x4 v = xr[i];
-#pragma unroll
-    for (int e = 0; e < 4; ++e) {
-      const float lo = __uint_as_float(v[e] << 16), hi = __uint_as_float(v[e] & 0xffff0000u);
-      s0 = fmaf(lo, lo, s0);
-      s1 = fmaf(hi, hi, s1);
-    }
-  }
-  const float t = wave_sum(s0 + s1);
-  if (lane == 0) inv[row] = 1.f / sqrtf(t / (float)D + eps);
+    rms_piece_acc(xr[i], s0, s1);
+  }
+  const float r = rms_row_inv(s0, s1, D, eps);
+  if (lane == 0) inv[row] = r;
 }
 
 int rms_rowinv(const bf16_t* x, float* inv, int M, int D, float eps, hipStream_t s) {
diff --git a/jax_llama_amd/models/llama.py b/jax_llama_amd/models/llama.py
--- a/jax_llama_amd/models/llama.py
+++ b/jax_llama_amd/models/llama.py
@@ -12,7 +12,7 @@
 from ..parallel.comm import NO_COMM, TPComm
 from ..parallel.partition import shard_tree
 from .kv_cache import KVCache
-from .modules import LLaMABlockCollection
+from .modules import LLaMABlockCollection, NormStat
 from .weights import Fp8Linear, PackedLinear
 
 BF16 = torch.bfloat16
@@ -301,9 +301,12 @@
                        self.head_dim, self.device)
 
     def _row_parallel(self, x: torch.Tensor, w: PackedLinear, h: torch.Tensor, hb: torch.Tensor,
-                      x_packed: Optional[torch.Tensor] = None, mirror_packed: Optional[torch.Tensor] = None) -> None:
+                      x_packed: Optional[torch.Tensor] = None, mirror_packed: Optional[torch.Tensor] = None,
+                      stat=None) -> None:
+        if stat is not None:
+            stat.clear()
         if self.comm.size == 1:
-            ops.linear_residual(x, w, h, mirror=hb, x_packed=x_packed, mirror_packed=mirror_packed)
+            ops.linear_residual(x, w, h, mirror=hb, x_packed=x_packed, mirror_packed=mirror_packed, stat=stat)
         elif self.comm.linear_residual_(x, w, h, hb, x_packed=x_packed, hb_pack=mirror_packed):
             pass
         else:
@@ -326,9 +329,11 @@
         b, s = ids.shape
         d = self.config.hidden_size
         hb = torch.empty(b * s, d, dtype=BF16, device=self.device)
+        stat = NormStat(b * s, self.eps, hb.device)
         h = ops.embedding(ids.reshape(-1), self.wte, mirror=hb)
+        stat.clear()
         hidden, attns = self.blocks(h, hb, positions, cache, slot0, kv_start, key_mask, s,
-                                    output_hidden_states=collect_hidden, output_attentions=collect_attn)
+                                    output_hidden_states=collect_hidden, output_attentions=collect_attn, stat=stat)
         if logits_mode == "none":
             logits = None
         elif logits_mode == "logprob":
@@ -343,10 +348,11 @@
             if logits_mode == "argmax":
                 logits = ops.argmax(logits.contiguous())
         elif logits_mode == "argmax":
-            logits = ops.linear_argmax(hb.reshape(b, s, d)[:, -1].contiguous(), self.lm_head, rms_eps=self.eps)
+            logits = ops.linear_argmax(hb.reshape(b, s, d)[:, -1].contiguous(), self.lm_head, rms_eps=self.eps,
+                                       stat=stat)
         else:
             hl = hb if logits_mode == "all" else hb.reshape(b, s, d)[:, -1].contiguous()
-            logits = ops.linear(hl, self.lm_head, rms_eps=self.eps, out_dtype=torch.float32)
+            logits = ops.linear(hl, self.lm_head, rms_eps=self.eps, out_dtype=torch.float32, stat=stat)
         return logits, h, hidden, attns
 
     def gather_logits(self, logits_local: torch.Tensor) -> torch.Tensor:
diff --git a/jax_llama_amd/models/modules.py b/jax_llama_amd/models/modules.py
--- a/jax_llama_amd/models/modules.py
+++ b/jax_llama_amd/models/modules.py
@@ -18,7 +18,8 @@
         return self.model.layers[self.layer_idx]
 
     def __call__(self, h, hb, positions, cache, slot0, kv_start, key_mask, seq_len: int,
-                 output_attentions: bool = False, pk: Optional["PackedActs"] = None) -> Optional[torch.Tensor]:
+                 output_attentions: bool = False, pk: Optional["PackedActs"] = None,
+                 stat: Optional["NormStat"] = None) -> Optional[torch.Tensor]:
         m, lw = self.model, self.weights
         kc, vc = cache.layer(self.layer_idx)
         splits = og = 0
@@ -39,12 +40,14 @@
                                          m.n_kv_heads, m.head_dim, splits, x_packed=pk.hb_in() if pk else None,
                                          out_packed=att_p, o=o)
             if not og:
-                m._row_parallel(a, lw.o, h, hb, x_packed=att_p, mirror_packed=hb_p)
+                m._row_parallel(a, lw.o, h, hb, x_packed=att_p, mirror_packed=hb_p, stat=stat)
+            elif stat is not None:
+                stat.clear()
             if pk is not None and pk.hb is not None:
                 pk.hb_ok = True
             return None
         q = ops.linear_qkv_rope(hb, lw.qkv, m.eps, m.rope, positions, kc, vc, slot0, seq_len,
-                                m.n_heads, m.n_kv_heads, m.head_dim, x_packed=pk.hb_in() if pk else None)
+                                m.n_heads, m.n_kv_heads, m.head_dim, x_packed=pk.hb_in() if pk else None, stat=stat)
         b = hb.shape[0] // seq_len
         q4 = q.reshape(b, seq_len, m.n_heads, m.head_dim)
         weights = None
@@ -56,7 +59,7 @@
         else:
             att_p = pk.att if pk is not None and ops.attention_packs(q4, kc, key_mask) else None
             a = ops.attention(q4, kc, vc, slot0, kv_start, key_mask, out_packed=att_p)
-        m._row_parallel(a, lw.o, h, hb, x_packed=att_p, mirror_packed=pk.hb if pk else None)
+        m._row_parallel(a, lw.o, h, hb, x_packed=att_p, mirror_packed=pk.hb if pk else None, stat=stat)
         if pk is not None and pk.hb is not None:
             pk.hb_ok = True
         return weights
@@ -67,12 +70,13 @@
         self.model = model
         self.layer_idx = layer_idx
 
-    def __call__(self, h, hb, pk: Optional["PackedActs"] = None) -> None:
+    def __call__(self, h, hb, pk: Optional["PackedActs"] = None, stat: Optional["NormStat"] = None) -> None:
         m, lw = self.model, self.model.layers[self.layer_idx]
         g = ops.linear_swiglu(hb, lw.gu, rms_eps=m.eps, x_packed=pk.hb_in() if pk else None,
-                              out_packed=pk.act if pk else None)
+                              out_packed=pk.act if pk else None, stat=stat)
 
-        m._row_parallel(g, lw.down, h, hb, x_packed=pk.act if pk else None, mirror_packed=pk.hb if pk else None)
+        m._row_parallel(g, lw.down, h, hb, x_packed=pk.act if pk else None, mirror_packed=pk.hb if pk else None,
+                        stat=stat)
 
 
 class LLaMABlock:
@@ -82,9 +86,10 @@
         self.feed_forward = LLaMAMLP(model, layer_idx)
 
     def __call__(self, h, hb, positions, cache, slot0, kv_start, key_mask, seq_len: int,
-                 output_attentions: bool = False, pk: Optional["PackedActs"] = None):
-        w = self.attention(h, hb, positions, cache, slot0, kv_start, key_mask, seq_len, output_attentions, pk)
-        self.feed_forward(h, hb, pk)
+                 output_attentions: bool = False, pk: Optional["PackedActs"] = None,
+                 stat: Optional["NormStat"] = None):
+        w = self.attention(h, hb, positions, cache, slot0, kv_start, key_mask, seq_len, output_attentions, pk, stat)
+        self.feed_forward(h, hb, pk, stat)
         return w
 
 
@@ -100,6 +105,26 @@
         return self.hb if self.hb_ok else None
 
 
+class NormStat:
+
+    def __init__(self, rows: int, eps: float, device):
+        self.eps = float(eps)
+        self.buf = ops.workspace.get("resid_stat", rows, torch.float32, device)
+        self.of: Optional[torch.Tensor] = None
+
+    def clear(self) -> None:
+        self.of = None
+
+    def mark(self, hb: torch.Tensor) -> None:
+        self.of = hb
+
+    def ready_for(self, x: torch.Tensor, eps) -> bool:
+        o = self.of
+        return (o is not None and eps is not None and float(eps) == self.eps
+                and x.dtype == o.dtype and x.shape == o.shape and x.data_ptr() == o.data_ptr()
+                and x.is_contiguous() and x.shape[0] <= self.buf.numel())
+
+
 class LLaMABlockCollection:
 
     def __init__(self, model):
@@ -110,7 +135,8 @@
         return len(self.blocks)
 
     def __call__(self, h, hb, positions, cache, slot0, kv_start, key_mask, seq_len: int,
-                 output_hidden_states: bool = False, output_attentions: bool = False):
+                 output_hidden_states: bool = False, output_attentions: bool = False,
+                 stat: Optional[NormStat] = None):
         hidden, attns = [], []
         b = hb.shape[0] // seq_len
         rows = hb.shape[0]
@@ -121,7 +147,7 @@
         for blk in self.blocks:
             if output_hidden_states:
                 hidden.append(h.reshape(b, seq_len, -1).clone())
-            w = blk(h, hb, positions, cache, slot0, kv_start, key_mask, seq_len, output_attentions, pk)
+            w = blk(h, hb, positions, cache, slot0, kv_start, key_mask, seq_len, output_attentions, pk, stat)
             if output_attentions:
                 attns.append(w)
         return hidden, attns
diff --git a/jax_llama_amd/ops/__init__.py b/jax_llama_amd/ops/__init__.py
--- a/jax_llama_amd/ops/__init__.py
+++ b/jax_llama_amd/ops/__init__.py
@@ -150,7 +150,7 @@
 
 
 def linear(x: torch.Tensor, w, rms_eps: Optional[float] = None, out_dtype=BF16,
-           out: Optional[torch.Tensor] = None, x_packed: Optional[torch.Tensor] = None) -> torch.Tensor:
+           out: Optional[torch.Tensor] = None, x_packed: Optional[torch.Tensor] = None, stat=None) -> torch.Tensor:
     if not _is_gpu(x):
         r = ref.linear(x, w.dense(), rms_eps, out_dtype)
         if out is not None:
@@ -160,28 +160,31 @@
     m = x.shape[0]
     if out is None:
         out = torch.empty(m, w.n, dtype=out_dtype, device=x.device)
-    _gpu_linear(x, w, out, MODE_STORE, rms_eps, True, None, x_packed)
+    _gpu_linear(x, w, out, MODE_STORE, rms_eps, True, None, x_packed, None, stat)
     return out
 
 
 def linear_residual(x: torch.Tensor, w, residual: torch.Tensor, rms_eps: Optional[float] = None,
                     accumulate: bool = True, mirror: Optional[torch.Tensor] = None,
-                    x_packed: Optional[torch.Tensor] = None, mirror_packed: Optional[torch.Tensor] = None) -> torch.Tensor:
+                    x_packed: Optional[torch.Tensor] = None, mirror_packed: Optional[torch.Tensor] = None,
+                    stat=None) -> torch.Tensor:
+    if stat is not None:
+        stat.clear()
     if not _is_gpu(x):
         ref.linear_residual(x, w.dense(), residual, rms_eps, accumulate)
         if mirror is not None:
             mirror.copy_(residual.to(BF16))
         return residual
-    _gpu_linear(x, w, residual, MODE_RESIDUAL, rms_eps, accumulate, mirror, x_packed, mirror_packed)
+    _gpu_linear(x, w, residual, MODE_RESIDUAL, rms_eps, accumulate, mirror, x_packed, mirror_packed, stat)
     return residual
 
 
 def linear_swiglu(x: torch.Tensor, w, rms_eps: Optional[float] = None, x_packed: Optional[torch.Tensor] = None,
-                  out_packed: Optional[torch.Tensor] = None) -> torch.Tensor:
+                  out_packed: Optional[torch.Tensor] = None, stat=None) -> torch.Tensor:
     if not _is_gpu(x):
         return ref.linear_swiglu(x, w.dense(), rms_eps)
     out = torch.empty(x.shape[0], w.n // 2, dtype=BF16, device=x.device)
-    _gpu_linear(x, w, out, MODE_SWIGLU, rms_eps, True, None, x_packed, out_packed)
+    _gpu_linear(x, w, out, MODE_SWIGLU, rms_eps, True, None, x_packed, out_packed, stat)
     return out
 
 
@@ -223,7 +226,7 @@
     return x.shape[0] > 0 and e.gemv_w8_plan_check(x.shape[0], w.n, w.k, mode, x.dtype != BF16)[0] == 0
 
 
-def _gpu_linear(x, w, out, mode, rms_eps, accumulate, mirror=None, x_packed=None, pack_out=None):
+def _gpu_linear(x, w, out, mode, rms_eps, accumulate, mirror=None, x_packed=None, pack_out=None, stat=None):
     assert x.is_contiguous() and out.is_contiguous()
     assert x.shape[1] == w.k, (x.shape, w.k)
     m = x.shape[0]
@@ -240,7 +243,7 @@
     if v == TILED and pack_out is not None and not _tiled_packs(e, m, w.n, w.k, x.device, mode, rms_eps):
         v = 1
     if v == TILED:
-        _tiled(e, x, w.weight, w.n, w.k, out, mode, rms_eps, accumulate, mirror, pack_out)
+        _tiled(e, x, w.weight, w.n, w.k, out, mode, rms_eps, accumulate, mirror, pack_out, stat)
     else:
         ws, tk = _skinny_ws(e, m, w.n, w.k, mode, x.device)
         e.linear_skinny(x, w.weight, w.n, w.k, out, mode, -1.0 if rms_eps is None else float(rms_eps),
@@ -304,12 +307,32 @@
     return workspace.get("gemm_rms", x.shape[0], torch.float32, x.device)
 
 
-def _tiled(e, x, weight, n, k, out, mode, rms_eps, accumulate, mirror=None, pack_out=None):
+RESIDUAL_STAT = True
+MODE_ARGMAX = 8
+NORM_PRECOMPUTED = 2
+
+
+def _stat_ws(e, x, stat, n, k, mode, fused: bool, ks: int, tm: int, rms_eps):
+    if (RESIDUAL_STAT and fused and stat is not None and stat.ready_for(x, rms_eps)
+            and e.gemm_plan_norm(x.shape[0], n, k, mode, True, ks, tm, True) == NORM_PRECOMPUTED):
+        return stat.buf, True
+    return _rms_ws(x, fused, ks), False
+
+
+def _tiled(e, x, weight, n, k, out, mode, rms_eps, accumulate, mirror=None, pack_out=None, stat=None):
     fused = _fused_rms(e, mode, rms_eps)
     xb = _tiled_input(x, rms_eps, fused)
     ks, tm, ws = _gemm_ws(e, x.shape[0], n, k, x.device, mode, fused)
+    if mode == MODE_RESIDUAL:
+        give = RESIDUAL_STAT and stat is not None and mirror is not None
+        wrote = e.gemm(xb, weight, n, k, out, mode, bool(accumulate), mirror, ks, ws, -1.0, tm, pack_out, None, 0,
+                       stat.buf if give else None, float(stat.eps) if give else 0.0, False)
+        if give and wrote:
+            stat.mark(mirror)
+        return
+    rws, ready = _stat_ws(e, x, stat, n, k, mode, fused, ks, tm, rms_eps)
     e.gemm(xb, weight, n, k, out, mode, bool(accumulate), mirror, ks, ws, float(rms_eps) if fused else -1.0, tm,
-           pack_out, _rms_ws(x, fused, ks))
+           pack_out, rws, 0, None, 0.0, ready)
 
 
 def _tiled_packs(e, m, n, k, device, mode, rms_eps) -> bool:
@@ -387,7 +410,7 @@
 
 def linear_qkv_rope(x: torch.Tensor, w, rms_eps: Optional[float], table: torch.Tensor, positions: torch.Tensor,
                     k_cache: torch.Tensor, v_cache: torch.Tensor, slot0, seq_len: int, n_heads: int,
-                    n_kv_heads: int, head_dim: int, x_packed: Optional[torch.Tensor] = None) -> torch.Tensor:
+                    n_kv_heads: int, head_dim: int, x_packed: Optional[torch.Tensor] = None, stat=None) -> torch.Tensor:
     if not _is_gpu(x):
         s0 = int(slot0) if not torch.is_tensor(slot0) else int(slot0.item())
         return ref.linear_qkv_rope(x, w.dense(), rms_eps, table, positions, k_cache, v_cache, s0, seq_len,
@@ -410,9 +433,10 @@
         fused = _fused_rms(e, MODE_QKV, rms_eps)
         if ks == 1 and fused and QKV_DIRECT and e.gemm_qkv_direct_ok(m, tm, w.k):
             q = torch.empty(m, n_heads, head_dim, dtype=BF16, device=x.device)
+            rws, ready = _stat_ws(e, x, stat, w.n, w.k, MODE_QKV, fused, 1, tm, rms_eps)
             e.gemm_qkv(_tiled_input(x, rms_eps, fused), w.weight, w.n, w.k, table, positions.reshape(-1).to(torch.int32),
                        k_cache, v_cache, _slot_tensor(slot0, x.device), int(seq_len), int(n_heads), int(n_kv_heads),
-                       int(head_dim), q, 1, None, float(rms_eps), tm, _rms_ws(x, fused, 1))
+                       int(head_dim), q, 1, None, float(rms_eps), tm, rws, ready)
             return q
         if ks == 1:
             qkv = linear(x, w, rms_eps=rms_eps)
@@ -571,7 +595,7 @@
 SKINNY_ARGMAX = os.environ.get("JLA_SKINNY_ARGMAX", "1") != "0"
 
 
-def linear_argmax(x: torch.Tensor, w, rms_eps: Optional[float] = None):
+def linear_argmax(x: torch.Tensor, w, rms_eps: Optional[float] = None, stat=None):
     m = x.shape[0]
     if not _is_gpu(x):
         return argmax(linear(x, w, rms_eps, out_dtype=torch.float32))
@@ -587,15 +611,15 @@
                                    val)
             return idx, val
     if m < ARGMAX_FUSED_MIN_M:
-        return argmax(linear(x, w, rms_eps, out_dtype=torch.float32))
+        return argmax(linear(x, w, rms_eps, out_dtype=torch.float32, stat=stat))
     e = ext()
     assert x.is_contiguous() and x.shape[1] == w.k, (x.shape, w.k)
     xb = x if x.dtype == BF16 else x.to(BF16)
     ws = workspace.get("gemm_argmax", e.gemm_argmax_workspace(m, w.n), torch.float32, x.device)
     idx = torch.empty(m, dtype=torch.int32, device=x.device)
     val = torch.empty(m, dtype=torch.float32, device=x.device)
-    e.gemm_argmax(xb, w.weight, w.n, w.k, ws, -1.0 if rms_eps is None else float(rms_eps), idx, val,
-                  _rms_ws(x, rms_eps is not None, 1))
+    rws, ready = _stat_ws(e, x, stat, w.n, w.k, MODE_ARGMAX, rms_eps is not None, 1, 0, rms_eps)
+    e.gemm_argmax(xb, w.weight, w.n, w.k, ws, -1.0 if rms_eps is None else float(rms_eps), idx, val, rws, ready)
     return idx, val
 
 
```

Result: no change. 42930 tokens/s, median of 6 (+0.3%).
